# akosiorek/attend_infer_repeat

Measured on AMD Instinct MI355X. Metric: images/sec (train step, ELBO backward) multi-MNIST 50x50, 3-step AIR, higher is better.
Workload: dtype f32; 1 GPU; multi-MNIST-shaped 50x50 canvas, max_steps=3, glimpse 20x20, batch=64 per GPU, fp32, hipGraph replay (BASELINE configs[1]); global_batch=64, batch_per_gpu=64, parallelism=dp1, hipgraph=True, steps_per_graph_replay=1, keep_canvas_steps=True, collective=none, dist_world_size=1, params_finite_after_run=True, replicas_in_sync_after_run=True

## Files before the change

### attend_infer_repeat_amd/csrc/air_common.h

```cpp
#pragma once
#include <hip/hip_runtime.h>
#include <stdint.h>
#include <stdlib.h>
#include <mutex>
#include "../../include/air_hip.h"

#define AIR_WAVE 64

#define AIR_REQUIRE(cond, code) do { if (!(cond)) return (code); } while (0)
#define AIR_LAUNCH_CHECK() do { hipError_t e__ = hipGetLastError(); if (e__ != hipSuccess) return (int)e__; } while (0)

static inline long air_gemm_wide_min_tiles() {
    static const long wide_min = getenv("AIR_GEMM_WIDE_MIN_TILES") ? atol(getenv("AIR_GEMM_WIDE_MIN_TILES")) : 1000;
    return wide_min;
}
static inline int air_gemm_latency_tile(long tiles16) { return tiles16 > 1536 ? 32 : 16; }
static inline bool air_gemm_long_k(int M, int N, int K) { return K >= 512 && K >= 8 * (M < N ? M : N); }
static inline bool air_gemm_lone_on_tile16_kw4(int M, int N, int K) {
    const long t = (long)((M + 15) / 16) * ((N + 15) / 16);
    return t <= air_gemm_wide_min_tiles() && air_gemm_latency_tile(t) == 16 && !air_gemm_long_k(M, N, K);
}

static inline hipStream_t air_stream(void *s) { return reinterpret_cast<hipStream_t>(s); }
static inline bool air_aligned16(const void *p) { return (reinterpret_cast<uintptr_t>(p) & 15u) == 0; }
__device__ __forceinline__ bool air_aligned16_dev(const void *p) { return (reinterpret_cast<uintptr_t>(p) & 15u) == 0; }
static inline int air_cdiv(long a, long b) { return (int)((a + b - 1) / b); }
static inline size_t air_rider_blocks(size_t nq, int nth, size_t cap) {
    static const double qpt = getenv("AIR_RIDER_QPT") ? atof(getenv("AIR_RIDER_QPT")) : 2.0;
    const double per_wg = (qpt > 0.05 ? qpt : 2.0) * nth;
    size_t extra = (size_t)(((double)nq + per_wg - 1.0) / per_wg);
    return extra > cap ? cap : extra;
}
template <typename K>
static inline int air_resident_grid(K kernel, int threads, size_t lds, int fallback) {
    struct Entry { const void *k; int threads; size_t lds; int dev; int grid; };
    static Entry cache[32];
    static int n_cached = 0;
    static std::mutex mu;
    int dev = 0;
    if (hipGetDevice(&dev) != hipSuccess) return fallback;
    const void *key = reinterpret_cast<const void *>(kernel);
    std::lock_guard<std::mutex> lock(mu);
    for (int i = 0; i < n_cached; ++i)
        if (cache[i].k == key && cache[i].threads == threads && cache[i].lds == lds && cache[i].dev == dev) return cache[i].grid;
    int per_cu = 0, cus = 0;
    if (hipDeviceGetAttribute(&cus, hipDeviceAttributeMultiprocessorCount, dev) != hipSuccess ||
        hipOccupancyMaxActiveBlocksPerMultiprocessor(&per_cu, kernel, threads, lds) != hipSuccess || per_cu < 1 || cus < 1)
        return fallback;
    if (n_cached < 32) cache[n_cached++] = Entry{key, threads, lds, dev, per_cu * cus};
    return per_cu * cus;
}

__device__ __forceinline__ int opaque_zero() {
    int z;
    asm volatile("v_mov_b32 %0, 0" : "=v"(z));
    return z;
}

__device__ __forceinline__ float wave_sum(float v) {
#pragma unroll
    for (int off = 32; off > 0; off >>= 1) v += __shfl_down(v, off, 64);
    return v;
}
__device__ __forceinline__ double wave_sum(double v) {
#pragma unroll
    for (int off = 32; off > 0; off >>= 1) v += __shfl_down(v, off, 64);
    return v;
}
__device__ __forceinline__ float wave_sum_all(float v) {
#pragma unroll
    for (int off = 32; off > 0; off >>= 1) v += __shfl_xor(v, off, 64);
    return v;
}
__device__ __forceinline__ double wave_sum_all(double v) {
#pragma unroll
    for (int off = 32; off > 0; off >>= 1) v += __shfl_xor(v, off, 64);
    return v;
}
__device__ __forceinline__ float wave_max_all(float v) {
#pragma unroll
    for (int off = 32; off > 0; off >>= 1) v = fmaxf(v, __shfl_xor(v, off, 64));
    return v;
}

template <typename T>
__device__ __forceinline__ T wave_reduce8(const T (&v)[8]) {
    const int lane = threadIdx.x & 63;
    const bool h5 = (lane & 32) != 0, h4 = (lane & 16) != 0, h3 = (lane & 8) != 0;
    T a[4], b[2];
#pragma unroll
    for (int i = 0; i < 4; ++i) a[i] = (h5 ? v[i + 4] : v[i]) + __shfl_xor(h5 ? v[i] : v[i + 4], 32, 64);
#pragma unroll
    for (int i = 0; i < 2; ++i) b[i] = (h4 ? a[i + 2] : a[i]) + __shfl_xor(h4 ? a[i] : a[i + 2], 16, 64);
    T c = (h3 ? b[1] : b[0]) + __shfl_xor(h3 ? b[0] : b[1], 8, 64);
    c += __shfl_xor(c, 4, 64);
    c += __shfl_xor(c, 2, 64);
    c += __shfl_xor(c, 1, 64);
    return c;
}
__device__ __forceinline__ int wave_reduce8_slot() {
    const int lane = threadIdx.x & 63;
    return ((lane >> 5) & 1) * 4 + ((lane >> 4) & 1) * 2 + ((lane >> 3) & 1);
}

template <int NV>
__device__ __forceinline__ void block_sum(float (&v)[NV], float *scratch) {
    const int lane = threadIdx.x & 63, wid = threadIdx.x >> 6, nw = (blockDim.x + 63) >> 6;
#pragma unroll
    for (int k = 0; k < NV; ++k) v[k] = wave_sum(v[k]);
    if (lane == 0) {
#pragma unroll
        for (int k = 0; k < NV; ++k) scratch[wid * NV + k] = v[k];
    }
    __syncthreads();
    if (wid == 0) {
#pragma unroll
        for (int k = 0; k < NV; ++k) {
            float x = lane < nw ? scratch[lane * NV + k] : 0.f;
            v[k] = wave_sum(x);
        }
    }
}

__device__ __forceinline__ float lin_m11(int k, int n, double step) {
#pragma clang fp contract(off)
    if (n <= 1) return -1.0f;
    if (k == n - 1) return 1.0f;
    const double prod = (double)k * step;
    return (float)(prod + -1.0);
}
__device__ __forceinline__ float grid_coord(float s, float X, float t, float half_extent) {
#pragma clang fp contract(off)
    const float a = s * X;
    const float b = a + t;
    const float c = b + 1.0f;
    return c * half_extent;
}
__device__ __forceinline__ float4 attention_box4(const float4 w4, float Wf, float Hf) {
#pragma clang fp contract(off)
    float4 bx;
    bx.x = Wf * ((1.f - w4.x) + w4.y) * 0.5f;
    bx.y = Hf * ((1.f - w4.z) + w4.w) * 0.5f;
    bx.z = Wf * w4.x;
    bx.w = Hf * w4.z;
    return bx;
}
__device__ __forceinline__ float sigmoidf_(float x) { return 1.0f / (1.0f + __expf(-x)); }
__device__ __forceinline__ float sigmoid_acc(float x) { return 1.0f / (1.0f + expf(-x)); }
__device__ __forceinline__ float softplus_acc(float x) { return x > 20.0f ? x : log1pf(expf(x)); }
__device__ __forceinline__ float elu_acc(float x) { return x > 0.0f ? x : expm1f(x); }
```

### attend_infer_repeat_amd/csrc/gemm_kernels.hip

```cpp
#include "air_common.h"
#include "prologue_device.h"
#include "optimizer_device.h"
#include "engine_device.h"
#include "nvil_device.h"
#include "gemm_device.h"
#include <cstring>
#include <type_traits>


struct AproArgs {
    const float *A2, *a_bias;
    float *a_out;
    int a_elu;
};
#define AIR_OPT_MAX_RANGES 4
struct OptFold {
    float *p; const float *g0; float *ms, *mg, *mom;
    size_t n_model;
    const float *lr_dev;
    float lr_mult_tail, decay, momentum, eps, gscale;
    unsigned fold_mask;
    int n_ranges, tiles;
    size_t lo[AIR_OPT_MAX_RANGES], hi[AIR_OPT_MAX_RANGES];
    int64_t *gstep; uint64_t *rng_state; uint64_t rng_inc;
};
#define AIR_OPT_RIDERS(OPT_)                                                                                                     \
    if ((int)blockIdx.x >= OPT_.tiles) {                                                                                         \
        const int vb = (int)blockIdx.x - OPT_.tiles, vg = (int)gridDim.x - OPT_.tiles;                                           \
        for (int r = 0; r < OPT_.n_ranges; ++r) {                                                                                \
            RmspropSlice sl;                                                                                                     \
            sl.p = OPT_.p; sl.g = OPT_.g0; sl.ms = OPT_.ms; sl.mg = OPT_.mg; sl.mom = OPT_.mom;                                  \
            sl.lo = OPT_.lo[r]; sl.hi = OPT_.hi[r]; sl.n_model = OPT_.n_model; sl.lr_dev = OPT_.lr_dev;                          \
            sl.lr_mult_tail = OPT_.lr_mult_tail; sl.decay = OPT_.decay; sl.momentum = OPT_.momentum; sl.eps = OPT_.eps;          \
            sl.gscale = OPT_.gscale;                                                                                             \
            rmsprop_slice_body(sl, vb, vg);                                                                                      \
        }                                                                                                                        \
        if (vb == 0 && threadIdx.x == 0) {                                                                                       \
            if (OPT_.gstep) OPT_.gstep[0] += 1;                                                                                  \
            if (OPT_.rng_state) OPT_.rng_state[1] += OPT_.rng_inc;                                                               \
        }                                                                                                                        \
        return;                                                                                                                  \
    }
struct GaussEpi {
    const float *pre, *eps, *loc, *scale, *dkl_row;
    float *dpre;
    int ld_pre, ld_dpre, D;
    float raw_offset, pl, ps, dkl_scale, guard;
    unsigned mask;
};
struct GatherArgs {
    const float *data, *obs;
    float *obs_out;
    long long n_items;
    int item_floats, shuffle, B;
    const uint64_t *seed;
    const int64_t *step;
    int64_t *idx_out;
    unsigned copy_mask;
};
__device__ __forceinline__ long long gather_item(const GatherArgs &gt, int m) {
    const unsigned long long ctr = (unsigned long long)gt.step[0] * (unsigned long long)gt.B + (unsigned long long)m;
    if (gt.shuffle) {
        uint32_t r[4];
        philox4x32(ctr, 1, gt.seed[0], r);
        const unsigned long long wide = ((unsigned long long)r[0] << 32) | r[1];
        return (long long)(((unsigned __int128)wide * (unsigned __int128)gt.n_items) >> 64);
    }
    return (long long)(ctr % (unsigned long long)gt.n_items);
}
struct GemmArgs {
    const float *A, *B, *bias, *aux;
    float *C, *colsum, *ws;
    int M, N, K, lda, ldb, ldc, ldaux;
    int ta, tb, epi, S, chunks_per_split, vecA, vecB;
    float beta;
};


__device__ __forceinline__ float apply_epilogue(float v, int m, int n, const GemmArgs &g) {
    if (g.beta != 0.f) v += g.beta * g.C[(size_t)m * g.ldc + n];
    switch (g.epi) {
        case AIR_EPI_BIAS: v += g.bias[n]; break;
        case AIR_EPI_BIAS_ELU: v = elu_acc(v + g.bias[n]); break;
        case AIR_EPI_MUL_DELU: {
            const float y = g.aux[(size_t)m * g.ldaux + n];
            v *= (y > 0.f ? 1.f : y + 1.f);
        } break;
        case AIR_EPI_ADD_AUX:
            v += g.aux[(size_t)m * g.ldaux + n];
            if (g.bias) v += g.bias[n];
            break;
        case AIR_EPI_ADD_AUX_ELU:
            v += g.aux[(size_t)m * g.ldaux + n];
            if (g.bias) v += g.bias[n];
            v = elu_acc(v);
            break;
        default: break;
    }
    return v;
}

template <int MT, int NT, int KW, bool BF, bool APRO = false, bool OPT = false, bool GBW = false, bool GATH = false>
__device__ __forceinline__ void gemm_body(const GemmArgs &g, const int block_tile, const int split, const AproArgs pro = AproArgs(),
                                          void *c16 = nullptr, const OptFold *opt = nullptr, const bool fold = false,
                                          const GaussEpi *gb = nullptr, const GatherArgs *gt = nullptr, const bool gcopy = false) {
    const gh_t hC = (gh_t)c16;
    constexpr int TM = 16 * MT, TN = 16 * NT;
    constexpr int NWN = (KW == 1) ? 4 : 1;
    constexpr int NWV = (KW == 1) ? 4 : KW;
    constexpr int NTH = 64 * NWV;
    constexpr int LDT = TN + 4;
    __shared__ float s_tile[NWV][TM * LDT];
    __shared__ float s_col[NWV][TN];

    const gcf gA = (gcf)g.A, gB = (gcf)g.B, gBias = (gcf)g.bias, gAux = (gcf)g.aux;
    const gf gC = (gf)g.C, gWs = (gf)g.ws, gCol = (gf)g.colsum;
    const int lane = threadIdx.x & 63, wave = threadIdx.x >> 6;
    const int li = lane & 15, lg = lane >> 4;
    const int tiles_n = (g.N + TN * NWN - 1) / (TN * NWN);
    const int tm = block_tile / tiles_n, tn = block_tile - tm * tiles_n;
    const int m0 = tm * TM;
    const int n0 = (tn * NWN + (KW == 1 ? wave : 0)) * TN;

    const int total_chunks = (g.K + 15) >> 4;
    const int c_begin = split * g.chunks_per_split;
    int c_end = c_begin + g.chunks_per_split;
    if (c_end > total_chunks) c_end = total_chunks;

    f32x4 acc[MT][NT];
#pragma unroll
    for (int a = 0; a < MT; ++a)
#pragma unroll
        for (int b = 0; b < NT; ++b) acc[a][b] = (f32x4){0.f, 0.f, 0.f, 0.f};
    float csum[NT];
#pragma unroll
    for (int b = 0; b < NT; ++b) csum[b] = 0.f;
    const bool want_colsum = (g.colsum != nullptr) && (tm == 0);

    int rowA[MT], colB[NT];
    bool okA[MT], okB[NT];
#pragma unroll
    for (int a = 0; a < MT; ++a) { rowA[a] = m0 + 16 * a + li; okA[a] = rowA[a] < g.M; }
#pragma unroll
    for (int b = 0; b < NT; ++b) { colB[b] = n0 + 16 * b + li; okB[b] = colB[b] < g.N; }

    constexpr int EPT = (KW > 1) ? (TM * TN + NTH - 1) / NTH : 1;
    float e_bias[EPT], e_aux[EPT], e_c[EPT];
    if (KW > 1 && g.S == 1) {
#pragma unroll
        for (int i = 0; i < EPT; ++i) {
            const int e = threadIdx.x + NTH * i;
            const int r = e / TN, cidx = e - r * TN;
            const int m = m0 + r, n = n0 + cidx;
            const bool ok = (e < TM * TN) && m < g.M && n < g.N;
            e_bias[i] = (ok && g.bias != nullptr) ? gBias[n] : 0.f;
            e_aux[i] = (ok && g.epi >= AIR_EPI_MUL_DELU) ? gAux[(size_t)m * g.ldaux + n] : 0.f;
            e_c[i] = (ok && g.beta != 0.f) ? gC[(size_t)m * g.ldc + n] : 0.f;
        }
    }
    float b_loc[GBW ? EPT : 1], b_scale[GBW ? EPT : 1], b_eps[GBW ? EPT : 1], b_raw[GBW ? EPT : 1], b_dk[GBW ? EPT : 1];
    if (GBW && KW > 1 && fold) {
#pragma unroll
        for (int i = 0; i < EPT; ++i) {
            const int e = threadIdx.x + NTH * i;
            const int r = e / TN, cidx = e - r * TN;
            const int m = m0 + r, n = n0 + cidx;
            const bool ok = (e < TM * TN) && m < g.M && n < g.N;
            const size_t o = ok ? (size_t)m * gb->D + n : 0;
            b_loc[i] = ok ? ((gcf)gb->loc)[o] : 0.f;
            b_scale[i] = ok ? ((gcf)gb->scale)[o] : 1.f;
            b_eps[i] = ok ? ((gcf)gb->eps)[o] : 0.f;
            b_raw[i] = ok ? ((gcf)gb->pre)[(size_t)m * gb->ld_pre + gb->D + n] : 0.f;
            b_dk[i] = (ok && gb->dkl_row) ? ((gcf)gb->dkl_row)[m] : 0.f;
        }
    }
    float o_p[OPT ? EPT : 1], o_ms[OPT ? EPT : 1], o_mg[OPT ? EPT : 1], o_mom[OPT ? EPT : 1];
    float o_lr0 = 0.f;
    if (OPT && KW > 1 && fold) {
        o_lr0 = ((gcf)opt->lr_dev)[0];
#pragma unroll
        for (int i = 0; i < EPT; ++i) {
            const int e = threadIdx.x + NTH * i;
            const int r = e / TN, cidx = e - r * TN;
            const int m = m0 + r, n = n0 + cidx;
            const bool ok = (e < TM * TN) && m < g.M && n < g.N;
            const size_t idx = ok ? (size_t)((gC + (size_t)m * g.ldc + n) - (gf)opt->g0) : 0;
            o_p[i] = ok ? ((gf)opt->p)[idx] : 0.f;
            o_ms[i] = ok ? ((gf)opt->ms)[idx] : 0.f;
            o_mg[i] = ok ? ((gf)opt->mg)[idx] : 0.f;
            o_mom[i] = ok ? ((gf)opt->mom)[idx] : 0.f;
        }
    }

    const int c_step = (KW > 1) ? KW : 1;
    int c = c_begin + ((KW > 1) ? wave : 0);
    constexpr int U = (MT * NT == 1) ? (KW == 16 ? 10 : 8) : 4;
    int full_end = g.K >> 4;
    if (full_end > c_end) full_end = c_end;
    int rowAc[MT], colBc[NT];
#pragma unroll
    for (int a = 0; a < MT; ++a) rowAc[a] = okA[a] ? rowA[a] : g.M - 1;
#pragma unroll
    for (int b = 0; b < NT; ++b) colBc[b] = okB[b] ? colB[b] : g.N - 1;
    const int gcol = GATH ? (int)(gA - (gcf)gt->obs) : 0;
    const gcf gAs = GATH ? (gcf)gt->data + gcol : gA;
    const int ldAs = GATH ? gt->item_floats : g.lda;
    int rowAs[MT];
#pragma unroll
    for (int a = 0; a < MT; ++a) rowAs[a] = GATH ? (int)gather_item(*gt, rowAc[a]) : rowAc[a];
    if (GATH && gcopy && tn == 0 && split == 0 && wave == 0 && lg == 0 && gt->idx_out && gcol == 0) {
#pragma unroll
        for (int a = 0; a < MT; ++a) if (okA[a]) gt->idx_out[rowA[a]] = rowAs[a];
    }
#pragma nounroll
    for (; c < full_end; c += U * c_step) {
        f32x4 fa[U][MT], fb[U][NT];
        f32x4 fa2[APRO ? U : 1][APRO ? MT : 1], fab[APRO ? U : 1];
#pragma unroll
        for (int u = 0; u < U; ++u) {
            const int cu = c + u * c_step;
            if (cu < full_end) {
                const int k = (cu << 4) + 4 * lg;
#pragma unroll
                for (int a = 0; a < MT; ++a) {
                    fa[u][a] = g.ta ? ld_kstrided_full(gA, g.lda, rowAc[a], k)
                                    : ld_kcontig_full(gAs, ldAs, rowAs[a], k, g.vecA != 0);
                    if (APRO) {
                        fa2[u][a] = ld_kcontig_full((gcf)pro.A2, g.lda, rowAc[a], k, g.vecA != 0);
                        fab[u] = ld_kcontig_full((gcf)pro.a_bias, 0, 0, k, g.vecA != 0);
                    }
                }
#pragma unroll
                for (int b = 0; b < NT; ++b)
                    fb[u][b] = g.tb ? ld_kcontig_full(gB, g.ldb, colBc[b], k, g.vecB != 0)
                                    : ld_kstrided_full(gB, g.ldb, colBc[b], k);
            } else {
#pragma unroll
                for (int a = 0; a < MT; ++a) fa[u][a] = (f32x4){0.f, 0.f, 0.f, 0.f};
#pragma unroll
                for (int b = 0; b < NT; ++b) fb[u][b] = (f32x4){0.f, 0.f, 0.f, 0.f};
            }
        }
#pragma unroll
        for (int u = 0; u < U; ++u) {
            if (c + u * c_step >= full_end) break;
            if (APRO) {
#pragma unroll
                for (int a = 0; a < MT; ++a) {
                    f32x4 v = (fa[u][a] + fa2[u][a]) + fab[u];
                    if (pro.a_elu) { v.x = elu_acc(v.x); v.y = elu_acc(v.y); v.z = elu_acc(v.z); v.w = elu_acc(v.w); }
                    fa[u][a] = v;
                    if (pro.a_out != nullptr && tn == 0 && okA[a])
                        *(f32x4 *)(pro.a_out + (size_t)rowA[a] * g.lda + (((c + u * c_step) << 4) + 4 * lg)) = v;
                }
            }
            if (GATH && gcopy && tn == 0) {
#pragma unroll
                for (int a = 0; a < MT; ++a)
                    if (okA[a]) *(f32x4 *)(gt->obs_out + (size_t)rowA[a] * g.lda + gcol + (((c + u * c_step) << 4) + 4 * lg)) = fa[u][a];
            }
            mfma_chunk<MT, NT, BF>(acc, fa[u], fb[u]);
            if (want_colsum) {
#pragma unroll
                for (int b = 0; b < NT; ++b)
                    csum[b] += okB[b] ? (fb[u][b].x + fb[u][b].y) + (fb[u][b].z + fb[u][b].w) : 0.f;
            }
        }
    }
    const int pc = g.K >> 4;
    if ((g.K & 15) && pc >= c_begin && pc < c_end && (KW == 1 || ((pc - c_begin) % KW) == wave)) {
        const int k = (pc << 4) + 4 * lg;
        f32x4 fa[MT], fb[NT];
#pragma unroll
        for (int a = 0; a < MT; ++a)
            fa[a] = g.ta ? ld_kstrided(gA, g.lda, rowA[a], okA[a], k, g.K)
                         : ld_kcontig(gAs, ldAs, GATH ? rowAs[a] : rowA[a], okA[a], k, g.K, g.vecA != 0);
        if (GATH && gcopy && tn == 0) {
#pragma unroll
            for (int a = 0; a < MT; ++a) {
                if (!okA[a]) continue;
                float *d = gt->obs_out + (size_t)rowA[a] * g.lda + gcol + k;
                if (k < g.K) d[0] = fa[a].x;
                if (k + 1 < g.K) d[1] = fa[a].y;
                if (k + 2 < g.K) d[2] = fa[a].z;
                if (k + 3 < g.K) d[3] = fa[a].w;
            }
        }
#pragma unroll
        for (int b = 0; b < NT; ++b)
            fb[b] = g.tb ? ld_kcontig(gB, g.ldb, colB[b], okB[b], k, g.K, g.vecB != 0)
                         : ld_kstrided(gB, g.ldb, colB[b], okB[b], k, g.K);
        mfma_chunk<MT, NT, BF>(acc, fa, fb);
        if (want_colsum) {
#pragma unroll
            for (int b = 0; b < NT; ++b) csum[b] += (fb[b].x + fb[b].y) + (fb[b].z + fb[b].w);
        }
    }

#pragma unroll
    for (int a = 0; a < MT; ++a)
#pragma unroll
        for (int b = 0; b < NT; ++b)
#pragma unroll
            for (int r = 0; r < 4; ++r) s_tile[wave][(16 * a + 4 * lg + r) * LDT + 16 * b + li] = acc[a][b][r];
    if (want_colsum) {
#pragma unroll
        for (int b = 0; b < NT; ++b) {
            float v = csum[b];
            v += __shfl_xor(v, 16, 64);
            v += __shfl_xor(v, 32, 64);
            if (lg == 0) s_col[wave][16 * b + li] = v;
        }
    }
    __syncthreads();

    if (KW > 1) {
#pragma unroll
        for (int i = 0; i < EPT; ++i) {
            const int e = threadIdx.x + NTH * i;
            if (e >= TM * TN) continue;
            const int r = e / TN, cidx = e - r * TN;
            const int m = m0 + r, n = n0 + cidx;
            if (m >= g.M || n >= g.N) continue;
            const int off = r * LDT + cidx;
            float v = 0.f;
#pragma unroll
            for (int q = 0; q < NWV; q += 4)
                v += (s_tile[q][off] + s_tile[q + 1][off]) + (s_tile[q + 2][off] + s_tile[q + 3][off]);
            if (g.S > 1) {
                gWs[((size_t)split * g.M + m) * g.N + n] = v;
            } else {
                if (g.beta != 0.f) v += g.beta * e_c[i];
                switch (g.epi) {
                    case AIR_EPI_BIAS: v += e_bias[i]; break;
                    case AIR_EPI_BIAS_ELU: v = elu_acc(v + e_bias[i]); break;
                    case AIR_EPI_MUL_DELU: v *= (e_aux[i] > 0.f ? 1.f : e_aux[i] + 1.f); break;
                    case AIR_EPI_ADD_AUX: v += e_aux[i] + e_bias[i]; break;
                    case AIR_EPI_ADD_AUX_ELU: v = elu_acc(v + e_aux[i] + e_bias[i]); break;
                    default: break;
                }
                gC[(size_t)m * g.ldc + n] = v;
                if (BF && hC) hC[(size_t)m * g.ldc + n] = bf16_bits(v);
                if (GBW && fold) {
                    float dloc, draw;
                    gauss_bwd_elem(v, true, b_eps[i], b_loc[i], b_scale[i], gb->pl, gb->ps, b_dk[i] * gb->dkl_scale,
                                   b_raw[i] + gb->raw_offset, 0, n, gb->guard, dloc, draw);
                    const gf dp_ = (gf)gb->dpre + (size_t)m * gb->ld_dpre;
                    dp_[n] = dloc; dp_[gb->D + n] = draw;
                }
                if (OPT && fold) {
                    const size_t idx = (size_t)((gC + (size_t)m * g.ldc + n) - (gf)opt->g0);
                    const float lr = idx < opt->n_model ? o_lr0 : o_lr0 * opt->lr_mult_tail;
                    float pv = o_p[i], a = o_ms[i], b = o_mg[i], c = o_mom[i];
                    rmsprop_elem(pv, v, a, b, c, lr, opt->decay, opt->momentum, opt->eps, opt->gscale);
                    ((gf)opt->ms)[idx] = a; ((gf)opt->mg)[idx] = b; ((gf)opt->mom)[idx] = c; ((gf)opt->p)[idx] = pv;
                }
            }
        }
        if (want_colsum && threadIdx.x < TN) {
            const int n = n0 + threadIdx.x;
            if (n < g.N) {
                float v = 0.f;
#pragma unroll
                for (int q = 0; q < NWV; q += 4)
                    v += (s_col[q][threadIdx.x] + s_col[q + 1][threadIdx.x]) + (s_col[q + 2][threadIdx.x] + s_col[q + 3][threadIdx.x]);
                gCol[n] = v;
                if (OPT && fold) {
                    const size_t idx = (size_t)((gCol + n) - (gf)opt->g0);
                    const float lr = idx < opt->n_model ? o_lr0 : o_lr0 * opt->lr_mult_tail;
                    float pv = ((gf)opt->p)[idx], a = ((gf)opt->ms)[idx], b = ((gf)opt->mg)[idx], c = ((gf)opt->mom)[idx];
                    rmsprop_elem(pv, v, a, b, c, lr, opt->decay, opt->momentum, opt->eps, opt->gscale);
                    ((gf)opt->ms)[idx] = a; ((gf)opt->mg)[idx] = b; ((gf)opt->mom)[idx] = c; ((gf)opt->p)[idx] = pv;
                }
            }
        }
    } else {
        for (int e = lane; e < TM * TN; e += 64) {
            const int r = e / TN, cidx = e - r * TN;
            const int m = m0 + r, n = n0 + cidx;
            if (m >= g.M || n >= g.N) continue;
            const float v = s_tile[wave][r * LDT + cidx];
            if (g.S > 1) gWs[((size_t)split * g.M + m) * g.N + n] = v;
            else {
                const float o = apply_epilogue(v, m, n, g);
                gC[(size_t)m * g.ldc + n] = o;
                if (BF && hC) hC[(size_t)m * g.ldc + n] = bf16_bits(o);
            }
        }
        if (want_colsum && lane < TN) {
            const int n = n0 + lane;
            if (n < g.N) gCol[n] = s_col[wave][lane];
        }
    }
}

template <int MT, int NT, int KW, bool BF>
__global__ __launch_bounds__(KW == 1 ? 256 : 64 * KW) void gemm_f32_mfma_kernel(GemmArgs g) {
    gemm_body<MT, NT, KW, BF>(g, blockIdx.x, blockIdx.y);
}
template <int MT, int NT, int KW>
__global__ __launch_bounds__(KW == 1 ? 256 : 64 * KW) void gemm_bf16_c16_kernel(GemmArgs g, void *c16) {
    gemm_body<MT, NT, KW, true>(g, blockIdx.x, blockIdx.y, AproArgs(), c16);
}
template <int MT, int NT, int KW, bool BF>
__global__ __launch_bounds__(KW == 1 ? 256 : 64 * KW) void gemm_f32_mfma_apro_kernel(GemmArgs g, AproArgs pro) {
    gemm_body<MT, NT, KW, BF, true>(g, blockIdx.x, blockIdx.y, pro);
}

template <int MT, int KW, bool BF, bool TA, bool TB>
__device__ __forceinline__ void gemm_wide_body(const GemmArgs &g, const int block_tile) {
    constexpr int NT = 4, TM = 16 * MT, TN = 64;
    constexpr int NTH = 64 * KW;
    constexpr int LDT = TN + 4;
    static_assert(!TA || MT == 4, "an m-contiguous A operand is read 4 rows per lane: four interleaved row tiles");
    __shared__ float s_tile[KW][TM * LDT];
    __shared__ float s_col[KW][TN];

    const gcf gA = (gcf)g.A, gB = (gcf)g.B, gBias = (gcf)g.bias, gAux = (gcf)g.aux;
    const gf gC = (gf)g.C, gCol = (gf)g.colsum;
    const int lane = threadIdx.x & 63, wave = threadIdx.x >> 6;
    const int li = lane & 15, lg = lane >> 4;
    const int tiles_n = (g.N + TN - 1) / TN;
    const int tm = block_tile / tiles_n, tn = block_tile - tm * tiles_n;
    const int m0 = tm * TM, n0 = tn * TN;

    f32x4 acc[MT][NT];
#pragma unroll
    for (int a = 0; a < MT; ++a)
#pragma unroll
        for (int b = 0; b < NT; ++b) acc[a][b] = (f32x4){0.f, 0.f, 0.f, 0.f};
    float csum[NT] = {0.f, 0.f, 0.f, 0.f};
    const bool want_colsum = TA && (g.colsum != nullptr) && (tm == 0);

    int offA[TA ? 1 : MT], offB[TB ? NT : 1];
    if (TA) { int r = m0 + 4 * li; if (r > g.M - 4) r = g.M - 4; offA[0] = r; }
    else {
#pragma unroll
        for (int a = 0; a < MT; ++a) { int r = m0 + 16 * a + li; if (r > g.M - 1) r = g.M - 1; offA[a] = r * g.lda; }
    }
    if (!TB) { int c = n0 + 4 * li; if (c > g.N - 4) c = g.N - 4; offB[0] = c; }
    else {
#pragma unroll
        for (int b = 0; b < NT; ++b) { int c = n0 + 16 * b + li; if (c > g.N - 1) c = g.N - 1; offB[b] = c * g.ldb; }
    }

    constexpr int EPT = (TM * TN) / NTH;
    static_assert((TM * TN) % NTH == 0, "tile / threads");
    float e_bias[EPT], e_aux[EPT], e_c[EPT];
#pragma unroll
    for (int i = 0; i < EPT; ++i) {
        const int e = threadIdx.x + NTH * i;
        const int r = e / TN, cidx = e - r * TN;
        int m = m0 + r, n = n0 + cidx;
        if (m > g.M - 1) m = g.M - 1;
        if (n > g.N - 1) n = g.N - 1;
        e_bias[i] = g.bias != nullptr ? gBias[n] : 0.f;
        e_aux[i] = g.epi >= AIR_EPI_MUL_DELU ? gAux[(size_t)m * g.ldaux + n] : 0.f;
        e_c[i] = g.beta != 0.f ? gC[(size_t)m * g.ldc + n] : 0.f;
    }

    constexpr int U = (MT == 4) ? 3 : 4;
    const int full_end = g.K >> 4;
    auto load_chunk = [&](int k, f32x4 (&fa)[MT], f32x4 (&fb)[NT]) {
        if (TA) {
            f32x4 v[4];
#pragma unroll
            for (int j = 0; j < 4; ++j) v[j] = *(gcf4)(gA + (size_t)(k + j) * g.lda + offA[0]);
#pragma unroll
            for (int a = 0; a < MT; ++a) fa[a] = (f32x4){v[0][a], v[1][a], v[2][a], v[3][a]};
        } else {
#pragma unroll
            for (int a = 0; a < MT; ++a) fa[a] = *(gcf4)(gA + offA[a] + k);
        }
        if (!TB) {
// ... 248 lines not shown
                }
            }
        } else {
#pragma unroll
            for (int b = 0; b < NT; ++b) {
                if (full) {
                    if (B16) fb[b] = *(gcu4)(hB + offB[b] + k);
                    else fb[b] = pk8(*(gcf4)(gB + offB[b] + k), *(gcf4)(gB + offB[b] + k + 4));
                } else {
                    float v[8];
#pragma unroll
                    for (int j = 0; j < 8; ++j)
                        v[j] = j < kn ? (B16 ? bf16_to_f32(hB[offB[b] + k + j]) : gB[offB[b] + k + j]) : 0.f;
                    fb[b] = (u32x4){pk_bf16(v[0], v[1]), pk_bf16(v[2], v[3]), pk_bf16(v[4], v[5]), pk_bf16(v[6], v[7])};
                }
            }
        }
    };
    auto mma = [&](const u32x4 (&fa)[MT], const u32x4 (&fb)[NT]) {
#pragma unroll
        for (int a = 0; a < MT; ++a)
#pragma unroll
            for (int b = 0; b < NT; ++b)
                acc[a][b] = __builtin_amdgcn_mfma_f32_16x16x32_bf16(__builtin_bit_cast(bf16x8, fa[a]), __builtin_bit_cast(bf16x8, fb[b]),
                                                                   acc[a][b], 0, 0, 0);
    };

    constexpr int U = (MT == 4) ? ((A16 && B16) ? 2 : 1) : 2;
    const int full_end = g.K >> 5;
    int c = wave;
#pragma nounroll
    for (; c < full_end; c += U * KW) {
        u32x4 fa[U][MT], fb[U][NT];
#pragma unroll
        for (int u = 0; u < U; ++u) {
            int cu = c + u * KW;
            if (cu > full_end - 1) cu = full_end - 1;
            load_chunk((cu << 5) + 8 * lg, 8, fa[u], fb[u], true, c + u * KW < full_end);
        }
#pragma unroll
        for (int u = 0; u < U; ++u) {
            if (c + u * KW >= full_end) break;
            mma(fa[u], fb[u]);
        }
    }
    if ((g.K & 31) && (full_end % KW) == wave) {
        const int k = (full_end << 5) + 8 * lg;
        int kn = g.K - k;
        kn = kn < 0 ? 0 : (kn > 8 ? 8 : kn);
        u32x4 fa[MT], fb[NT];
        load_chunk(kn > 0 ? k : 0, kn, fa, fb, false, true);
        mma(fa, fb);
    }

#pragma unroll
    for (int a = 0; a < MT; ++a)
#pragma unroll
        for (int r = 0; r < 4; ++r) {
            const int row = TA ? 4 * (4 * lg + r) + a : 16 * a + 4 * lg + r;
            if (!TB) {
                *(f32x4 *)&s_tile[wave][row * LDT + 4 * li] = (f32x4){acc[a][0][r], acc[a][1][r], acc[a][2][r], acc[a][3][r]};
            } else {
#pragma unroll
                for (int b = 0; b < NT; ++b) s_tile[wave][row * LDT + 16 * b + li] = acc[a][b][r];
            }
        }
    if (want_colsum) {
#pragma unroll
        for (int b = 0; b < NT; ++b) {
            float v = csum[b];
            v += __shfl_xor(v, 16, 64);
            v += __shfl_xor(v, 32, 64);
            if (lg == 0) s_col[wave][TB ? 16 * b + li : 4 * li + b] = v;
        }
    }
    __syncthreads();
#pragma unroll
    for (int i = 0; i < EPT; ++i) {
        const int e = threadIdx.x + NTH * i;
        const int r = e / TN, cidx = e - r * TN;
        const int m = m0 + r, n = n0 + cidx;
        const int off = r * LDT + cidx;
        float v = 0.f;
#pragma unroll
        for (int q = 0; q < KW; q += 4) v += (s_tile[q][off] + s_tile[q + 1][off]) + (s_tile[q + 2][off] + s_tile[q + 3][off]);
        if (g.beta != 0.f) v += g.beta * e_c[i];
        switch (g.epi) {
            case AIR_EPI_BIAS: v += e_bias[i]; break;
            case AIR_EPI_BIAS_ELU: v = elu_acc(v + e_bias[i]); break;
            case AIR_EPI_MUL_DELU: v *= (e_aux[i] > 0.f ? 1.f : e_aux[i] + 1.f); break;
            case AIR_EPI_ADD_AUX: v += e_aux[i] + e_bias[i]; break;
            case AIR_EPI_ADD_AUX_ELU: v = elu_acc(v + e_aux[i] + e_bias[i]); break;
            default: break;
        }
        if (m < g.M && n < g.N) {
            gC[(size_t)m * g.ldc + n] = v;
            if (hC) hC[(size_t)m * g.ldc + n] = bf16_bits(v);
        }
    }
    if (want_colsum && threadIdx.x < TN) {
        const int n = n0 + threadIdx.x;
        if (n < g.N) {
            float v = 0.f;
#pragma unroll
            for (int q = 0; q < KW; q += 4)
                v += (s_col[q][threadIdx.x] + s_col[q + 1][threadIdx.x]) + (s_col[q + 2][threadIdx.x] + s_col[q + 3][threadIdx.x]);
            gCol[n] = v;
        }
    }
}
template <int MT, int KW, bool TA, bool TB, bool A16, bool B16>
__global__ __launch_bounds__(64 * KW) void gemm_wide16_kernel(GemmArgs g, Gemm16Ptrs h) {
    __shared__ Wide16Lds<MT, KW> lds;
    gemm_wide16_body<MT, KW, TA, TB, A16, B16>(g, h, blockIdx.x, lds);
}

#define AIR_GEMM_GROUP_MAX 8
struct GroupArgs {
    GemmArgs g[AIR_GEMM_GROUP_MAX];
    int tile_start[AIR_GEMM_GROUP_MAX + 1];
    int count;
    int xcd_map;
    unsigned sk_mask;
};
#define AIR_GROUP_LOCATE(P_, GA_, VB_)                                                                                           \
    int P_ = 0;                                                                                                                  \
    _Pragma("unroll")                                                                                                            \
    for (int i = 1; i < AIR_GEMM_GROUP_MAX; ++i)                                                                                 \
        if (i < GA_.count && VB_ >= GA_.tile_start[i]) P_ = i;                                                                   \
    P_ = __builtin_amdgcn_readfirstlane(P_)
#define AIR_GROUP_SWITCH(P_, CASE_)                                                                                              \
    switch (P_) {                                                                                                                \
        case 0: CASE_(0); break;                                                                                                 \
        case 1: CASE_(1); break;                                                                                                 \
        case 2: CASE_(2); break;                                                                                                 \
        case 3: CASE_(3); break;                                                                                                 \
        case 4: CASE_(4); break;                                                                                                 \
        case 5: CASE_(5); break;                                                                                                 \
        case 6: CASE_(6); break;                                                                                                 \
        default: CASE_(7); break;                                                                                                \
    }
#define AIR_GROUP_DISPATCH(GA_, VB_, CASE_)                                                                                      \
    do {                                                                                                                         \
        AIR_GROUP_LOCATE(p, GA_, VB_);                                                                                           \
        AIR_GROUP_SWITCH(p, CASE_);                                                                                              \
    } while (0)
template <int MT, int NT, int KW, bool BF>
__global__ __launch_bounds__(KW == 1 ? 256 : 64 * KW) void gemm_grouped_kernel(GroupArgs ga) {
#define AIR_GG_CASE(I_) gemm_body<MT, NT, KW, BF>(ga.g[I_], (int)blockIdx.x - ga.tile_start[I_], blockIdx.y)
    AIR_GROUP_DISPATCH(ga, (int)blockIdx.x, AIR_GG_CASE);
#undef AIR_GG_CASE
}

__global__ __launch_bounds__(1024) void gemm_grouped_gather_kernel(GroupArgs ga, GatherArgs gt) {
#define AIR_GG_CASE(I_)                                                                                                             \
    gemm_body<1, 1, 16, false, false, false, false, true>(ga.g[I_], (int)blockIdx.x - ga.tile_start[I_], blockIdx.y, AproArgs(), nullptr, \
                                                          nullptr, false, nullptr, &gt, cp)
    AIR_GROUP_LOCATE(p, ga, (int)blockIdx.x);
    const bool cp = (gt.copy_mask >> p) & 1u;
    AIR_GROUP_SWITCH(p, AIR_GG_CASE);
#undef AIR_GG_CASE
}

template <int MT, int NT, int KW, bool BF>
__global__ __launch_bounds__(KW == 1 ? 256 : 64 * KW) void gemm_grouped_opt_kernel(GroupArgs ga, OptFold opt) {
    AIR_OPT_RIDERS(opt);
#define AIR_OPT_CASE(I_)                                                                                                          \
    gemm_body<MT, NT, KW, BF, false, true>(ga.g[I_], (int)blockIdx.x - ga.tile_start[I_], blockIdx.y, AproArgs(), nullptr, &opt,  \
                                           ((opt.fold_mask >> I_) & 1u) != 0)
    AIR_GROUP_DISPATCH(ga, (int)blockIdx.x, AIR_OPT_CASE);
#undef AIR_OPT_CASE
}

template <bool OPT>
__device__ __forceinline__ void shortk_dw_body(const GemmArgs &g, const int vb, const int vg, const OptFold *opt, const bool fold) {
    const gcf gA = (gcf)g.A, gB = (gcf)g.B;
    const gf gC = (gf)g.C, gCol = (gf)g.colsum;
    const int lane = threadIdx.x & 63, wave = threadIdx.x >> 6, li = lane & 15, lg = lane >> 4;
    const int n_base = 64 * wave;
    if (n_base >= g.N) return;
    const int nch = g.K >> 4;
    f32x4 fb[4][4];
#pragma unroll
    for (int c = 0; c < 4; ++c)
#pragma unroll
        for (int t = 0; t < 4; ++t)
            fb[c][t] = c < nch ? ld_kstrided_full(gB, g.ldb, n_base + 16 * t + li, (c << 4) + 4 * lg) : (f32x4){0.f, 0.f, 0.f, 0.f};
    float o_lr0 = 0.f;
    if (OPT && fold) o_lr0 = ((gcf)opt->lr_dev)[0];
    if (gCol != nullptr && vb == 0) {
#pragma unroll
        for (int t = 0; t < 4; ++t) {
            float v = 0.f;
#pragma unroll
            for (int c = 0; c < 4; ++c) v += (fb[c][t].x + fb[c][t].y) + (fb[c][t].z + fb[c][t].w);
            v += __shfl_xor(v, 16, 64);
            v += __shfl_xor(v, 32, 64);
            if (lg == 0) {
                const int n = n_base + 16 * t + li;
                gCol[n] = v;
                if (OPT && fold) {
                    const size_t idx = (size_t)((gCol + n) - (gf)opt->g0);
                    const float lr = idx < opt->n_model ? o_lr0 : o_lr0 * opt->lr_mult_tail;
                    float pv = ((gf)opt->p)[idx], a = ((gf)opt->ms)[idx], b = ((gf)opt->mg)[idx], cmo = ((gf)opt->mom)[idx];
                    rmsprop_elem(pv, v, a, b, cmo, lr, opt->decay, opt->momentum, opt->eps, opt->gscale);
                    ((gf)opt->ms)[idx] = a; ((gf)opt->mg)[idx] = b; ((gf)opt->mom)[idx] = cmo; ((gf)opt->p)[idx] = pv;
                }
            }
        }
    }
    const int tiles_m = (g.M + 15) >> 4;
    int mt = vb;
    if (mt >= tiles_m) return;
    f32x4 fa[4];
    {
        int m = (mt << 4) + li; if (m > g.M - 1) m = g.M - 1;
#pragma unroll
        for (int c = 0; c < 4; ++c) fa[c] = c < nch ? ld_kstrided_full(gA, g.lda, m, (c << 4) + 4 * lg) : (f32x4){0.f, 0.f, 0.f, 0.f};
    }
#pragma nounroll
    for (; mt < tiles_m; mt += vg) {
        f32x4 fn[4];
        {
            int mn = ((mt + vg) << 4) + li; if (mn > g.M - 1) mn = g.M - 1;
#pragma unroll
            for (int c = 0; c < 4; ++c) fn[c] = c < nch ? ld_kstrided_full(gA, g.lda, mn, (c << 4) + 4 * lg) : (f32x4){0.f, 0.f, 0.f, 0.f};
        }
        const int mrow0 = (mt << 4) + 4 * lg;
        f32x4 o_p[4], o_ms[4], o_mg[4], o_mom[4];
#pragma unroll
        for (int t = 0; t < 4; ++t) { o_p[t] = (f32x4){0.f, 0.f, 0.f, 0.f}; o_ms[t] = o_p[t]; o_mg[t] = o_p[t]; o_mom[t] = o_p[t]; }
        if (OPT && fold) {
#pragma unroll
            for (int r = 0; r < 4; ++r) {
                int mr = mrow0 + r; if (mr > g.M - 1) mr = g.M - 1;
                const size_t idx0 = (size_t)((gC + (size_t)mr * g.ldc + n_base + li) - (gf)opt->g0);
#pragma unroll
                for (int t = 0; t < 4; ++t) {
                    o_p[t][r] = ((gf)opt->p)[idx0 + 16 * t]; o_ms[t][r] = ((gf)opt->ms)[idx0 + 16 * t];
                    o_mg[t][r] = ((gf)opt->mg)[idx0 + 16 * t]; o_mom[t][r] = ((gf)opt->mom)[idx0 + 16 * t];
                }
            }
        }
        f32x4 acc[4];
#pragma unroll
        for (int t = 0; t < 4; ++t) acc[t] = (f32x4){0.f, 0.f, 0.f, 0.f};
#pragma unroll
        for (int c = 0; c < 4; ++c)
#pragma unroll
            for (int j = 0; j < 4; ++j)
#pragma unroll
                for (int t = 0; t < 4; ++t) acc[t] = __builtin_amdgcn_mfma_f32_16x16x4f32(fa[c][j], fb[c][t][j], acc[t], 0, 0, 0);
#pragma unroll
        for (int t = 0; t < 4; ++t)
#pragma unroll
            for (int r = 0; r < 4; ++r) {
                const int mr = mrow0 + r;
                if (mr < g.M) {
                    const size_t off = (size_t)mr * g.ldc + n_base + 16 * t + li;
                    const float v = acc[t][r];
                    gC[off] = v;
                    if (OPT && fold) {
                        const size_t idx = (size_t)((gC + off) - (gf)opt->g0);
                        const float lr = idx < opt->n_model ? o_lr0 : o_lr0 * opt->lr_mult_tail;
                        float pv = o_p[t][r], a = o_ms[t][r], b = o_mg[t][r], cmo = o_mom[t][r];
                        rmsprop_elem(pv, v, a, b, cmo, lr, opt->decay, opt->momentum, opt->eps, opt->gscale);
                        ((gf)opt->ms)[idx] = a; ((gf)opt->mg)[idx] = b; ((gf)opt->mom)[idx] = cmo; ((gf)opt->p)[idx] = pv;
                    }
                }
            }
#pragma unroll
        for (int c = 0; c < 4; ++c) fa[c] = fn[c];
    }
}
static inline bool shortk_eligible(const AirGemmDesc &d) {
    static const int on = getenv("AIR_GEMM_SHORTK") ? atoi(getenv("AIR_GEMM_SHORTK")) : 1;
    static const int min_m = getenv("AIR_GEMM_SHORTK_MIN_M") ? atoi(getenv("AIR_GEMM_SHORTK_MIN_M")) : 4096;
    return on && d.ta && !d.tb && d.precision == AIR_PREC_F32 && d.K >= 16 && d.K <= 64 && d.K % 16 == 0 && d.N >= 64 && d.N <= 256 &&
           d.N % 64 == 0 && d.M >= min_m && d.epilogue == AIR_EPI_NONE && d.beta == 0.f && !d.A2 && !d.C16 && !d.bias;
}
static inline int shortk_workgroups(int M) {
    static const int cap = getenv("AIR_GEMM_SHORTK_WGS") ? atoi(getenv("AIR_GEMM_SHORTK_WGS")) : 384;
    const int t = air_cdiv(M, 16);
    return t < cap ? t : (cap < 1 ? 1 : cap);
}

template <int MT, int NT>
__global__ __launch_bounds__(256) void gemm_grouped_sk_kernel(GroupArgs ga) {
#define AIR_SK_CASE(I_)                                                                                                        \
    do {                                                                                                                       \
        if ((ga.sk_mask >> I_) & 1u)                                                                                           \
            shortk_dw_body<false>(ga.g[I_], (int)blockIdx.x - ga.tile_start[I_], ga.tile_start[I_ + 1] - ga.tile_start[I_], nullptr, false); \
        else gemm_body<MT, NT, 4, false>(ga.g[I_], (int)blockIdx.x - ga.tile_start[I_], blockIdx.y);                           \
    } while (0)
    AIR_GROUP_DISPATCH(ga, (int)blockIdx.x, AIR_SK_CASE);
#undef AIR_SK_CASE
}
__global__ __launch_bounds__(256) void gemm_grouped_opt_sk_kernel(GroupArgs ga, OptFold opt) {
    AIR_OPT_RIDERS(opt);
#define AIR_SK_CASE(I_)                                                                                                        \
    shortk_dw_body<true>(ga.g[I_], (int)blockIdx.x - ga.tile_start[I_], ga.tile_start[I_ + 1] - ga.tile_start[I_], &opt,        \
                         ((opt.fold_mask >> I_) & 1u) != 0)
    AIR_GROUP_DISPATCH(ga, (int)blockIdx.x, AIR_SK_CASE);
#undef AIR_SK_CASE
}

// ... 203 lines not shown
    gemm_single_form(M, N, K, colsum != nullptr, ws != nullptr, ws_bytes, f);
    g.S = f.S; g.chunks_per_split = f.chunks_per_split;
    hipStream_t st = air_stream(stream);
    if (f.KW == 1) return launch_gemm<2, 2, 1, BF>(g, st);
    return launch_gemm<1, 1, 4, BF>(g, st);
}

extern "C" int air_gemm(int ta, int tb, int M, int N, int K, const float *A, int lda, const float *B, int ldb,
                        float *C, int ldc, const float *bias, int epilogue, const float *aux, int ldaux, float beta,
                        float *colsum, void *ws, size_t ws_bytes, void *stream) {
    return gemm_dispatch<false>(ta, tb, M, N, K, A, lda, B, ldb, C, ldc, bias, epilogue, aux, ldaux, beta, colsum, ws,
                                ws_bytes, stream);
}
extern "C" int air_gemm_bf16(int ta, int tb, int M, int N, int K, const float *A, int lda, const float *B, int ldb,
                             float *C, int ldc, const float *bias, int epilogue, const float *aux, int ldaux, float beta,
                             float *colsum, void *ws, size_t ws_bytes, void *stream) {
    return gemm_dispatch<true>(ta, tb, M, N, K, A, lda, B, ldb, C, ldc, bias, epilogue, aux, ldaux, beta, colsum, ws,
                               ws_bytes, stream);
}

static int fill_gemm_args(GemmArgs &g, const AirGemmDesc &d) {
    AIR_REQUIRE(d.A && d.B && d.C, AIR_E_NULL);
    AIR_REQUIRE(d.M > 0 && d.N > 0 && d.K > 0, AIR_E_SHAPE);
    AIR_REQUIRE(d.lda >= (d.ta ? d.M : d.K) && d.ldb >= (d.tb ? d.K : d.N) && d.ldc >= d.N, AIR_E_SHAPE);
    AIR_REQUIRE(d.epilogue >= AIR_EPI_NONE && d.epilogue <= AIR_EPI_ADD_AUX_ELU, AIR_E_UNSUPPORTED);
    if (d.epilogue == AIR_EPI_BIAS || d.epilogue == AIR_EPI_BIAS_ELU) AIR_REQUIRE(d.bias, AIR_E_NULL);
    if (d.epilogue >= AIR_EPI_MUL_DELU) AIR_REQUIRE(d.aux && d.ldaux >= d.N, AIR_E_NULL);
    AIR_REQUIRE(!d.colsum || d.ta, AIR_E_UNSUPPORTED);
    if (d.A2) {
        AIR_REQUIRE(!d.ta && d.a_bias && (d.K % 16 == 0) && (d.lda % 4 == 0), AIR_E_UNSUPPORTED);
        AIR_REQUIRE(air_aligned16(d.A) && air_aligned16(d.A2) && air_aligned16(d.a_bias) && (!d.a_out || air_aligned16(d.a_out)),
                    AIR_E_ALIGN);
    }
    g.A = d.A; g.B = d.B; g.C = d.C; g.bias = d.bias; g.aux = d.aux; g.colsum = d.colsum; g.ws = nullptr;
    g.M = d.M; g.N = d.N; g.K = d.K; g.lda = d.lda; g.ldb = d.ldb; g.ldc = d.ldc; g.ldaux = d.ldaux;
    g.ta = d.ta ? 1 : 0; g.tb = d.tb ? 1 : 0; g.epi = d.epilogue; g.beta = d.beta;
    g.vecA = (!d.ta && (d.lda % 4 == 0) && air_aligned16(d.A)) ? 1 : 0;
    g.vecB = (d.tb && (d.ldb % 4 == 0) && air_aligned16(d.B)) ? 1 : 0;
    g.S = 1; g.chunks_per_split = (d.K + 15) / 16;
    return AIR_OK;
}

template <class GA, class Tiles>
static int group_tile_starts(GA &ga, const AirGemmDesc *descs, int count, Tiles tiles_of) {
    constexpr int MAX = (int)(sizeof(ga.g) / sizeof(ga.g[0]));
    int tiles = 0;
    for (int i = 0; i < count; ++i) {
        ga.tile_start[i] = tiles;
        const int t = tiles_of(i, descs[i]);
        if (t < 0) return t;
        tiles += t;
    }
    for (int i = count; i <= MAX; ++i) ga.tile_start[i] = tiles;
    return tiles;
}
static int accept_any(int, const AirGemmDesc &) { return AIR_OK; }
template <class GA, class Accept, class Tiles>
static int fill_group(GA &ga, const AirGemmDesc *descs, int count, Accept accept, Tiles tiles_of, int *total) {
    constexpr int MAX = (int)(sizeof(ga.g) / sizeof(ga.g[0]));
    const int tiles = group_tile_starts(ga, descs, count, [&](int i, const AirGemmDesc &d) {
        int st = accept(i, d);
        if (st == AIR_OK) st = fill_gemm_args(ga.g[i], d);
        return st ? st : tiles_of(i, d);
    });
    if (tiles < 0) return tiles;
    for (int i = count; i < MAX; ++i) ga.g[i] = ga.g[0];
    ga.count = count;
    ga.xcd_map = 0;
    if constexpr (std::is_same<GA, GroupArgs>::value) ga.sk_mask = 0;
    *total = tiles;
    return AIR_OK;
}
template <class GA16, class GA, class Mirrors>
static void group_to16(GA16 &g16, const GA &ga, Mirrors mirrors_of) {
    constexpr int MAX = (int)(sizeof(ga.g) / sizeof(ga.g[0]));
    for (int i = 0; i < MAX; ++i) {
        const int j = i < ga.count ? i : 0;
        g16.g[i] = ga.g[j];
        g16.h[i] = mirrors_of(j);
    }
    for (int i = 0; i <= MAX; ++i) g16.tile_start[i] = ga.tile_start[i];
    g16.count = ga.count; g16.xcd_map = ga.xcd_map;
}
static bool bf16_storage() {
    static const int use16 = getenv("AIR_GEMM_BF16_STORAGE") ? atoi(getenv("AIR_GEMM_BF16_STORAGE")) : 1;
    return use16 != 0;
}
static inline bool mirror_usable(const void *m16, int ld) { return m16 && ld % 2 == 0 && ((uintptr_t)m16 % 4 == 0); }

static long group_tiles16(const AirGemmDesc *descs, int count, unsigned skip_mask) {
    long tiles16 = 0;
    for (int i = 0; i < count; ++i)
        if (!((skip_mask >> i) & 1u)) tiles16 += (long)air_cdiv(descs[i].M, 16) * air_cdiv(descs[i].N, 16);
    return tiles16;
}
static inline int latency_tile(long tiles16) { return air_gemm_latency_tile(tiles16); }
static bool group_long_k(const AirGemmDesc *descs, int count, long tiles16) {
    bool long_k = tiles16 <= 1024;
    for (int i = 0; i < count; ++i) long_k = long_k && air_gemm_long_k(descs[i].M, descs[i].N, descs[i].K);
    return long_k;
}
static int problem_precision(const AirGemmDesc &d, bool bf) {
    AIR_REQUIRE(d.precision == AIR_PREC_F32 || d.precision == AIR_PREC_BF16, AIR_E_UNSUPPORTED);
    AIR_REQUIRE((d.precision == AIR_PREC_BF16) == bf, AIR_E_UNSUPPORTED);
    return AIR_OK;
}
static int group_precision(const AirGemmDesc *descs, int count, bool *bf) {
    *bf = descs[0].precision == AIR_PREC_BF16;
    for (int i = 0; i < count; ++i)
        if (int st = problem_precision(descs[i], *bf)) return st;
    return AIR_OK;
}

static long wide_min_tiles() { return air_gemm_wide_min_tiles(); }
static bool group_on_long_k_body(const AirGemmDesc *descs, int count, long tiles16) {
    return tiles16 <= wide_min_tiles() && group_long_k(descs, count, tiles16);
}
static bool wide_group_eligible(const AirGemmDesc *descs, int count, long tiles16, bool bf, int *min_k_out, bool *nt_short_out) {
    static const long wide_tn_bf = getenv("AIR_GEMM_WIDE_TN_BF16") ? atol(getenv("AIR_GEMM_WIDE_TN_BF16")) : 48;
    static const long wide_tn_f32 = getenv("AIR_GEMM_WIDE_TN_F32") ? atol(getenv("AIR_GEMM_WIDE_TN_F32")) : 48;
    static const long wide_nt_k = getenv("AIR_GEMM_WIDE_NT_K") ? atol(getenv("AIR_GEMM_WIDE_NT_K")) : 512;
    bool ok = tiles16 > wide_min_tiles();
    const int ta = descs[0].ta ? 1 : 0, tb = descs[0].tb ? 1 : 0;
    long tiles64 = 0;
    int min_k = 1 << 30;
    for (int i = 0; i < count && ok; ++i) {
        const AirGemmDesc &d = descs[i];
        ok = ok && (d.ta ? 1 : 0) == ta && (d.tb ? 1 : 0) == tb && !(ta && tb) && !d.A2;
        ok = ok && air_aligned16(d.B) && d.ldb % 4 == 0 && (!ta || d.K % 4 == 0) && (!tb || d.K % 4 == 0);
        ok = ok && d.M >= 4 && d.N >= 4 && d.K >= 4 && (!ta || d.M % 4 == 0) && (tb || d.N % 4 == 0);
        if (tiles16 <= 2048) ok = ok && air_aligned16(d.A) && d.lda % 4 == 0 && d.K % 4 == 0;
        tiles64 += (long)air_cdiv(d.M, 64) * air_cdiv(d.N, 64);
        if (d.K < min_k) min_k = d.K;
    }
    if (ok && ta) ok = tiles64 >= (bf ? wide_tn_bf : wide_tn_f32) && min_k >= 256;
    const bool nt_short = !ta && tb && min_k < wide_nt_k;
    if (ok && nt_short) ok = bf && tiles16 > 2048;
    *min_k_out = min_k; *nt_short_out = nt_short;
    return ok;
}
static bool wide_regime_weight_gradients(const AirGemmDesc *descs, int count, long tiles16) {
    int min_k = 1 << 30;
    bool all_tn = true;
    for (int i = 0; i < count; ++i) { all_tn = all_tn && descs[i].ta && !descs[i].tb; if (descs[i].K < min_k) min_k = descs[i].K; }
    return tiles16 > wide_min_tiles() && all_tn && min_k >= 256;
}

static int validate_group(const AirGemmDesc *descs, int count) {
    GemmArgs scratch;
    for (int i = 0; i < count; ++i)
        if (int st = fill_gemm_args(scratch, descs[i])) return st;
    return AIR_OK;
}
static int form_workgroups_of(const AirGemmForm &f, int i, const AirGemmDesc &d) {
    switch (f.family) {
        case AIR_GEMM_FAM_BIG: case AIR_GEMM_FAM_BIG16:
            return ((f.small_mask >> i) & 1u) ? air_cdiv(d.M, 16) * air_cdiv(d.N, 16) : air_cdiv(d.M, 64) * air_cdiv(d.N, 64);
        case AIR_GEMM_FAM_WIDE: case AIR_GEMM_FAM_WIDE16:
            return air_cdiv(d.M, 16 * f.MT) * air_cdiv(d.N, 64);
        case AIR_GEMM_FAM_SHORTK:
            if ((f.sk_mask >> i) & 1u) return shortk_workgroups(d.M);
            [[fallthrough]];
        default:
            return air_cdiv(d.M, f.tile) * air_cdiv(d.N, f.tile);
    }
}
static void form_sum_workgroups(AirGemmForm &f, const AirGemmDesc *descs, int count) {
    f.workgroups = 0;
    for (int i = 0; i < count; ++i) f.workgroups += form_workgroups_of(f, i, descs[i]);
}
static int big_tn_form(const AirGemmDesc *descs, int count, AirGemmForm &f) {
    AIR_REQUIRE(count <= AIR_GEMM_BIG_GROUP_MAX, AIR_E_SHAPE);
    const bool bf = descs[0].precision == AIR_PREC_BF16;
    int min_k = 1 << 30, n_wide = 0;
    GemmArgs scratch;
    for (int i = 0; i < count; ++i) {
        const AirGemmDesc &d = descs[i];
        if (int e = problem_precision(d, bf)) return e;
        AIR_REQUIRE(!d.A2, AIR_E_UNSUPPORTED);
        if (int e = fill_gemm_args(scratch, d)) return e;
        const bool wide = d.ta && !d.tb && air_aligned16(d.B) && d.ldb % 4 == 0 && d.K % 4 == 0 && d.M >= 4 && d.N >= 4 &&
                          d.M % 4 == 0 && d.N % 4 == 0;
        if (wide) {
            if (d.K < min_k) min_k = d.K;
            ++n_wide;
        } else f.small_mask |= 1u << i;
        if (bf && bf16_storage() && mirror_usable(d.A16, d.lda)) f.a16_mask |= 1u << i;
        if (bf && bf16_storage() && mirror_usable(d.B16, d.ldb)) f.b16_mask |= 1u << i;
    }
    AIR_REQUIRE(n_wide > 0, AIR_E_UNSUPPORTED);
    static const int big_xcd = getenv("AIR_GEMM_BIG_XCD") ? atoi(getenv("AIR_GEMM_BIG_XCD")) : 1;
    f.xcd_map = (big_xcd && min_k >= 1024) ? (bf ? 2 : 1) : 0;
    f.family = bf ? AIR_GEMM_FAM_BIG16 : AIR_GEMM_FAM_BIG;
    f.grouped = 1; f.MT = 4; f.KW = 8; f.bf = bf ? 1 : 0; f.ta = 1; f.tb = 0;
    f.threads = 512;
    form_sum_workgroups(f, descs, count);
    return AIR_OK;
}
static int launch_big_tn_group(const AirGemmDesc *descs, int count, const AirGemmForm &f, void *stream) {
    BigGroupArgs ga;
    int wt = 0;
    int st = fill_group(ga, descs, count, accept_any, [&](int i, const AirGemmDesc &d) { return form_workgroups_of(f, i, d); }, &wt);
    if (st) return st;
    ga.small_mask = f.small_mask;
    ga.xcd_map = f.xcd_map;
    hipStream_t stm = air_stream(stream);
    if (f.family == AIR_GEMM_FAM_BIG16) {
        BigGroupArgs16 g16;
        group_to16(g16, ga, [&](int j) {
            const AirGemmDesc &d = descs[j];
            return Gemm16Ptrs{((f.a16_mask >> j) & 1u) ? d.A16 : nullptr, ((f.b16_mask >> j) & 1u) ? d.B16 : nullptr, nullptr};
        });
        g16.small_mask = ga.small_mask;
        hipLaunchKernelGGL((gemm_big_group_wide16_tn_kernel<4, 8>), dim3(wt), dim3(512), 0, stm, g16);
    } else hipLaunchKernelGGL((gemm_big_group_wide_tn_kernel<4, 8, false>), dim3(wt), dim3(512), 0, stm, ga);
    AIR_LAUNCH_CHECK();
    return AIR_OK;
}

static unsigned shortk_mask(const AirGemmDesc *descs, int count) {
    unsigned m = 0;
    for (int i = 0; i < count; ++i) {
        if (descs[i].A2 || descs[i].C16 || descs[i].precision != AIR_PREC_F32) return 0;
        if (shortk_eligible(descs[i])) m |= 1u << i;
    }
    return m;
}
static int launch_grouped_sk(const AirGemmDesc *descs, int count, const AirGemmForm &f, void *stream) {
    GroupArgs ga;
    int tiles = 0;
    int err = fill_group(ga, descs, count, accept_any, [&](int i, const AirGemmDesc &d) { return form_workgroups_of(f, i, d); }, &tiles);
    if (err) return err;
    ga.sk_mask = f.sk_mask;
    hipStream_t st = air_stream(stream);
    if (f.MT == 1) hipLaunchKernelGGL((gemm_grouped_sk_kernel<1, 1>), dim3(tiles), dim3(256), 0, st, ga);
    else hipLaunchKernelGGL((gemm_grouped_sk_kernel<2, 2>), dim3(tiles), dim3(256), 0, st, ga);
    AIR_LAUNCH_CHECK();
    return AIR_OK;
}

extern "C" int air_gemm_grouped_gather_fits(const AirGemmDesc *descs, int count, const AirBatchGather *g) {
    if (!descs || !g || count < 1 || count > AIR_GEMM_GROUP_MAX) return 0;
    if (!g->dataset || !g->obs || !g->seed_dev || !g->step_dev || g->n_items <= 0 || g->item_floats <= 0 || g->B <= 0) return 0;
    if (g->item_floats % 4 || !air_aligned16(g->dataset) || !air_aligned16(g->obs)) return 0;
    long tiles16 = 0;
    for (int i = 0; i < count; ++i) {
        const AirGemmDesc &d = descs[i];
        if (d.ta || d.A2 || d.C16 || d.precision != AIR_PREC_F32 || d.M != g->B || d.lda != g->item_floats) return 0;
        const long off = (const float *)d.A - (const float *)g->obs;
        if (off < 0 || off + d.K > g->item_floats || off % 4) return 0;
        tiles16 += (long)air_cdiv(d.M, 16) * air_cdiv(d.N, 16);
    }
    return group_on_long_k_body(descs, count, tiles16) ? 1 : 0;
}
extern "C" int air_gemm_grouped_gather(const AirGemmDesc *descs, int count, const AirBatchGather *g, void *stream) {
    AIR_REQUIRE(descs && g, AIR_E_NULL);
    AIR_REQUIRE(air_gemm_grouped_gather_fits(descs, count, g) == 1, AIR_E_UNSUPPORTED);
    GroupArgs ga;
    int tiles = 0;
    int err = fill_group(ga, descs, count, accept_any, [&](int i, const AirGemmDesc &d) {
        ga.g[i].vecA = 1;
        return air_cdiv(d.M, 16) * air_cdiv(d.N, 16);
    }, &tiles);
    if (err) return err;
    const GatherArgs gt = {g->dataset, g->obs, g->obs, g->n_items, g->item_floats, g->shuffle ? 1 : 0, g->B, g->seed_dev, g->step_dev,
                           g->idx_out, g->copy_mask};
    hipLaunchKernelGGL(gemm_grouped_gather_kernel, dim3(tiles), dim3(1024), 0, air_stream(stream), ga, gt);
    AIR_LAUNCH_CHECK();
    return AIR_OK;
}

static int gemm_grouped_form(const AirGemmDesc *descs, int count, AirGemmForm &f) {
    memset(&f, 0, sizeof f);
    if (count > AIR_GEMM_GROUP_MAX) return big_tn_form(descs, count, f);
    AIR_REQUIRE(count > 0 && count <= AIR_GEMM_GROUP_MAX, AIR_E_SHAPE);
    f.grouped = count > 1 ? 1 : 0;
    if (const unsigned skm = shortk_mask(descs, count)) {
        if (int err = validate_group(descs, count)) return err;
        f.family = AIR_GEMM_FAM_SHORTK; f.grouped = 1; f.sk_mask = skm;
        f.tile = latency_tile(group_tiles16(descs, count, skm));
        f.MT = f.NT = f.tile == 16 ? 1 : 2; f.KW = 4; f.threads = 256;
        form_sum_workgroups(f, descs, count);
        return AIR_OK;
    }
    const long tiles16 = group_tiles16(descs, count, 0u);
    const int T_ = latency_tile(tiles16);
    if (int err = validate_group(descs, count)) return err;
    const bool long_k = group_long_k(descs, count, tiles16);
    bool bf;
    if (int err = group_precision(descs, count, &bf)) return err;
    f.bf = bf ? 1 : 0;
    {
        const int ta = descs[0].ta ? 1 : 0, tb = descs[0].tb ? 1 : 0;
        int min_k;
        bool nt_short;
        const bool ok = wide_group_eligible(descs, count, tiles16, bf, &min_k, &nt_short);
        if (ok && bf && ta) {
            memset(&f, 0, sizeof f);
            return big_tn_form(descs, count, f);
        }
        if (ok) {
            f.family = bf ? AIR_GEMM_FAM_WIDE16 : AIR_GEMM_FAM_WIDE;
            f.ta = ta; f.tb = tb; f.nt_short = nt_short ? 1 : 0;
            f.MT = ta ? 4 : (nt_short ? 2 : 1); f.KW = 8; f.threads = 512;
            form_sum_workgroups(f, descs, count);
            f.xcd_map = (ta && min_k >= 1024) ? 1 : 0;
            if (bf) {
                bool a16 = bf16_storage(), b16 = bf16_storage();
                for (int i = 0; i < count; ++i) {
                    a16 = a16 && mirror_usable(descs[i].A16, descs[i].lda);
                    b16 = b16 && mirror_usable(descs[i].B16, descs[i].ldb);
                }
                f.a16_mask = a16 ? (1u << count) - 1u : 0u;
                f.b16_mask = b16 ? (1u << count) - 1u : 0u;
            }
            return AIR_OK;
        }
    }
    for (int i = 0; i < count; ++i) AIR_REQUIRE(!descs[i].A2 || count == 1, AIR_E_UNSUPPORTED);
    bool any_c16 = false;
    for (int i = 0; i < count; ++i) any_c16 = any_c16 || (descs[i].C16 != nullptr);
    f.tile = T_; f.long_k = long_k ? 1 : 0;
    f.MT = f.NT = (long_k || T_ == 16) ? 1 : 2; f.KW = long_k ? 16 : 4; f.threads = 64 * f.KW;
    if (any_c16) {
        AIR_REQUIRE(bf && !descs[0].A2, AIR_E_UNSUPPORTED);
        f.family = AIR_GEMM_FAM_C16;
    } else if (count == 1 && descs[0].A2) {
        AIR_REQUIRE(T_ == 16, AIR_E_UNSUPPORTED);
        f.family = AIR_GEMM_FAM_APRO; f.MT = f.NT = 1; f.KW = 4; f.threads = 256;
    } else f.family = AIR_GEMM_FAM_TILE;
    form_sum_workgroups(f, descs, count);
    return AIR_OK;
}
extern "C" int air_gemm_grouped_form(const AirGemmDesc *descs, int count, AirGemmForm *out) {
    AIR_REQUIRE(descs && out, AIR_E_NULL);
    return gemm_grouped_form(descs, count, *out);
}

extern "C" int air_gemm_grouped(const AirGemmDesc *descs, int count, void *stream) {
    AIR_REQUIRE(descs, AIR_E_NULL);
    AirGemmForm f;
    if (int err = gemm_grouped_form(descs, count, f)) return err;
    if (f.family == AIR_GEMM_FAM_BIG || f.family == AIR_GEMM_FAM_BIG16) return launch_big_tn_group(descs, count, f, stream);
    if (f.family == AIR_GEMM_FAM_SHORTK) return launch_grouped_sk(descs, count, f, stream);
    GroupArgs ga;
    int tiles = 0;
    const bool wide = f.family == AIR_GEMM_FAM_WIDE || f.family == AIR_GEMM_FAM_WIDE16;
    int err = fill_group(ga, descs, count, accept_any, [&](int i, const AirGemmDesc &d) { return form_workgroups_of(f, i, d); }, &tiles);
    if (err) return err;
    hipStream_t st = air_stream(stream);
    const bool bf = f.bf != 0;
    if (wide) {
        const int wt = tiles;
        ga.xcd_map = f.xcd_map;
        if (bf) {
            const bool a16 = f.a16_mask != 0u, b16 = f.b16_mask != 0u;
            GroupArgs16 g16;
            group_to16(g16, ga, [&](int j) {
                return Gemm16Ptrs{a16 ? descs[j].A16 : nullptr, b16 ? descs[j].B16 : nullptr, descs[j].C16};
            });
#define AIR_WIDE16_LAUNCH2(MT_, TA_, TB_, A16_, B16_)                                                                              \
            do {                                                                                                           \
                if (!f.grouped) hipLaunchKernelGGL((gemm_wide16_kernel<MT_, 8, TA_, TB_, A16_, B16_>), dim3(wt), dim3(512), 0, st, g16.g[0], g16.h[0]); \
                else hipLaunchKernelGGL((gemm_grouped_wide16_kernel<MT_, 8, TA_, TB_, A16_, B16_>), dim3(wt), dim3(512), 0, st, g16);                   \
            } while (0)
#define AIR_WIDE16_LAUNCH(MT_, TA_, TB_)                                                                                   \
            do {                                                                                                           \
                if (a16 && b16) AIR_WIDE16_LAUNCH2(MT_, TA_, TB_, true, true);                                             \
                else if (a16) AIR_WIDE16_LAUNCH2(MT_, TA_, TB_, true, false);                                              \
                else if (b16) AIR_WIDE16_LAUNCH2(MT_, TA_, TB_, false, true);                                              \
                else AIR_WIDE16_LAUNCH2(MT_, TA_, TB_, false, false);                                                      \
            } while (0)
            if (f.MT == 4) AIR_WIDE16_LAUNCH(4, true, false);
            else if (f.MT == 2) AIR_WIDE16_LAUNCH(2, false, true);
            else if (f.tb) AIR_WIDE16_LAUNCH(1, false, true);
            else AIR_WIDE16_LAUNCH(1, false, false);
#undef AIR_WIDE16_LAUNCH
#undef AIR_WIDE16_LAUNCH2
            AIR_LAUNCH_CHECK();
            return AIR_OK;
        }
#define AIR_WIDE_LAUNCH(MT_, TA_, TB_)                                                                                     \
        do {                                                                                                               \
            if (!f.grouped) hipLaunchKernelGGL((gemm_wide_kernel<MT_, 8, false, TA_, TB_>), dim3(wt), dim3(512), 0, st, ga.g[0]);         \
            else hipLaunchKernelGGL((gemm_grouped_wide_kernel<MT_, 8, false, TA_, TB_>), dim3(wt), dim3(512), 0, st, ga);                 \
        } while (0)
        if (f.MT == 4) AIR_WIDE_LAUNCH(4, true, false);
        else if (f.MT == 2) AIR_WIDE_LAUNCH(2, false, true);
        else if (f.tb) AIR_WIDE_LAUNCH(1, false, true);
        else AIR_WIDE_LAUNCH(1, false, false);
#undef AIR_WIDE_LAUNCH
        AIR_LAUNCH_CHECK();
        return AIR_OK;
    }
#define AIR_TILE_FORMS(LAUNCH_)                                                                                      \
    do {                                                                                                             \
        if (f.KW == 16) LAUNCH_(1, 1, 16, 1024);                                                                     \
        else if (f.MT == 1) LAUNCH_(1, 1, 4, 256);                                                                   \
        else LAUNCH_(2, 2, 4, 256);                                                                                  \
    } while (0)
#define AIR_GROUP_LAUNCH(MT_, NT_, KW_, NTH_)                                                                        \
    do {                                                                                                             \
        if (bf) hipLaunchKernelGGL((gemm_grouped_kernel<MT_, NT_, KW_, true>), dim3(tiles), dim3(NTH_), 0, st, ga);   \
        else hipLaunchKernelGGL((gemm_grouped_kernel<MT_, NT_, KW_, false>), dim3(tiles), dim3(NTH_), 0, st, ga);     \
    } while (0)
#define AIR_SINGLE_LAUNCH(MT_, NT_, KW_, NTH_)                                                                       \
    do {                                                                                                             \
        if (bf) hipLaunchKernelGGL((gemm_f32_mfma_kernel<MT_, NT_, KW_, true>), dim3(tiles, 1), dim3(NTH_), 0, st, ga.g[0]);  \
        else hipLaunchKernelGGL((gemm_f32_mfma_kernel<MT_, NT_, KW_, false>), dim3(tiles, 1), dim3(NTH_), 0, st, ga.g[0]);    \
    } while (0)
    if (f.family == AIR_GEMM_FAM_C16) {
        C16Ptrs c16;
        for (int i = 0; i < AIR_GEMM_GROUP_MAX; ++i) c16.p[i] = i < count ? descs[i].C16 : nullptr;
#define AIR_C16_LAUNCH(MT_, NT_, KW_, NTH_)                                                                          \
        do {                                                                                                         \
            if (!f.grouped) hipLaunchKernelGGL((gemm_bf16_c16_kernel<MT_, NT_, KW_>), dim3(tiles, 1), dim3(NTH_), 0, st, ga.g[0], c16.p[0]);  \
            else hipLaunchKernelGGL((gemm_grouped_c16_kernel<MT_, NT_, KW_>), dim3(tiles), dim3(NTH_), 0, st, ga, c16);                     \
        } while (0)
        AIR_TILE_FORMS(AIR_C16_LAUNCH);
#undef AIR_C16_LAUNCH
    } else if (f.family == AIR_GEMM_FAM_APRO) {
        const AproArgs pro = {descs[0].A2, descs[0].a_bias, descs[0].a_out, descs[0].a_elu};
        if (bf) hipLaunchKernelGGL((gemm_f32_mfma_apro_kernel<1, 1, 4, true>), dim3(tiles, 1), dim3(256), 0, st, ga.g[0], pro);
        else hipLaunchKernelGGL((gemm_f32_mfma_apro_kernel<1, 1, 4, false>), dim3(tiles, 1), dim3(256), 0, st, ga.g[0], pro);
    } else if (!f.grouped) AIR_TILE_FORMS(AIR_SINGLE_LAUNCH);
    else AIR_TILE_FORMS(AIR_GROUP_LAUNCH);
#undef AIR_SINGLE_LAUNCH
#undef AIR_GROUP_LAUNCH
#undef AIR_TILE_FORMS
    AIR_LAUNCH_CHECK();
    return AIR_OK;
}

extern "C" int air_gemm_grouped_gauss_bwd(const AirGemmDesc *descs, int count, const AirGaussBwdEpi *e, const float *imp_parts,
                                          int n_parts, float *imp_sum, const float *baseline, const float *logp, float *nvil_out,
                                          float *dlogp, float *dbaseline, int B, float *ema_dev, const float *kl_parts,
                                          int n_kl_parts, float *kl_row_out, int kl_rows, void *stream) {
    AIR_REQUIRE(descs && e, AIR_E_NULL);
    AIR_REQUIRE(count > 0 && count <= AIR_GEMM_GROUP_MAX && e->problem >= 0 && e->problem < count, AIR_E_SHAPE);
    AIR_REQUIRE(e->pre && e->eps && e->loc && e->scale && e->dpre && e->D > 0 && e->ld_pre >= 2 * e->D && e->ld_dpre >= 2 * e->D, AIR_E_NULL);
    AIR_REQUIRE(!imp_parts || (baseline && logp && nvil_out && B > 0 && n_parts > 0), AIR_E_NULL);
    AIR_REQUIRE(n_kl_parts >= 0 && (n_kl_parts == 0 || (kl_parts && kl_row_out && kl_rows > 0)), AIR_E_NULL);
    {
        const AirGemmDesc &d = descs[e->problem];
        AIR_REQUIRE(d.N == e->D && d.beta == 0.f && d.epilogue == AIR_EPI_NONE && !d.colsum, AIR_E_UNSUPPORTED);
    }
    GroupArgs ga;
    const long tiles16 = group_tiles16(descs, count, 0u);
    AIR_REQUIRE(tiles16 <= 1000, AIR_E_UNSUPPORTED);
    int tiles = 0;
    const bool bf = descs[0].precision == AIR_PREC_BF16;
    int err = fill_group(ga, descs, count,
        [&](int, const AirGemmDesc &d) -> int {
            if (int e = problem_precision(d, bf)) return e;
            AIR_REQUIRE(!d.A2 && !d.C16, AIR_E_UNSUPPORTED);
            return AIR_OK;
        },
        [&](int, const AirGemmDesc &d) { return air_cdiv(d.M, 16) * air_cdiv(d.N, 16); }, &tiles);
    if (err) return err;
    const bool long_k = group_long_k(descs, count, tiles16);
    GaussEpi gb;
    gb.pre = e->pre; gb.eps = e->eps; gb.loc = e->loc; gb.scale = e->scale; gb.dkl_row = e->dkl_row; gb.dpre = e->dpre;
    gb.ld_pre = e->ld_pre; gb.ld_dpre = e->ld_dpre; gb.D = e->D; gb.raw_offset = e->raw_offset; gb.pl = e->p_loc; gb.ps = e->p_scale;
    gb.dkl_scale = e->dkl_scale; gb.guard = e->guard_eps; gb.mask = 1u << e->problem;
    const NvilArgs nv = {imp_parts, baseline, logp, nvil_out, dlogp, dbaseline, B, n_parts > 0 ? n_parts : 1, imp_sum, ema_dev};
    const KlParts kp = {kl_parts, kl_row_out, n_kl_parts};
    const int riders = (imp_parts ? 1 : 0) + (n_kl_parts > 0 ? 1 : 0);
    hipStream_t st = air_stream(stream);
#define AIR_GB_LAUNCH(KW_, NTH_)                                                                                                   \
    do {                                                                                                                           \
        if (bf) hipLaunchKernelGGL((gemm_grouped_gb_kernel<1, 1, KW_, true>), dim3(tiles + riders), dim3(NTH_), 0, st, ga, gb, nv, kp, tiles, kl_rows);  \
        else hipLaunchKernelGGL((gemm_grouped_gb_kernel<1, 1, KW_, false>), dim3(tiles + riders), dim3(NTH_), 0, st, ga, gb, nv, kp, tiles, kl_rows);   \
    } while (0)
    if (long_k) AIR_GB_LAUNCH(16, 1024); else AIR_GB_LAUNCH(4, 256);
#undef AIR_GB_LAUNCH
    AIR_LAUNCH_CHECK();
    return AIR_OK;
}

extern "C" int air_gemm_grouped_opt(const AirGemmDesc *descs, int count, const AirOptFold *o, void *stream) {
    AIR_REQUIRE(descs && o, AIR_E_NULL);
    AIR_REQUIRE(count > 0 && count <= AIR_GEMM_GROUP_MAX, AIR_E_SHAPE);
    AIR_REQUIRE(o->p && o->g && o->ms && o->mg && o->mom && o->lr_dev, AIR_E_NULL);
    AIR_REQUIRE(o->n_ranges >= 0 && o->n_ranges <= AIR_OPT_MAX_RANGES && o->n_model % 4 == 0, AIR_E_SHAPE);
    AIR_REQUIRE(air_aligned16(o->p) && air_aligned16(o->g) && air_aligned16(o->ms) && air_aligned16(o->mg) && air_aligned16(o->mom), AIR_E_ALIGN);
    GroupArgs ga;
    const unsigned sk_mask = shortk_mask(descs, count);
    AIR_REQUIRE(sk_mask == 0 || sk_mask == (1u << count) - 1u, AIR_E_UNSUPPORTED);
    const long tiles16 = group_tiles16(descs, count, sk_mask);
    const int T_ = latency_tile(tiles16);
    int tiles = 0;
    const bool bf = descs[0].precision == AIR_PREC_BF16;
    int err = fill_group(ga, descs, count,
        [&](int, const AirGemmDesc &d) -> int {
            if (int e = problem_precision(d, bf)) return e;
            AIR_REQUIRE(!d.A2 && !d.C16, AIR_E_UNSUPPORTED);
            return AIR_OK;
        },
        [&](int i, const AirGemmDesc &d) -> int {
            if ((o->fold_mask >> i) & 1u) {
                AIR_REQUIRE(d.beta == 0.f && d.epilogue == AIR_EPI_NONE, AIR_E_UNSUPPORTED);
                AIR_REQUIRE(d.C >= o->g && (!d.colsum || d.colsum >= o->g), AIR_E_SHAPE);
            }
            return ((sk_mask >> i) & 1u) ? shortk_workgroups(d.M) : air_cdiv(d.M, T_) * air_cdiv(d.N, T_);
// ... 75 lines not shown
```

### attend_infer_repeat_amd/csrc/lstm_kernels.hip

```cpp
#include "air_common.h"
#include "prologue_device.h"
#include "optimizer_device.h"
#include "engine_device.h"
#include "nvil_device.h"
#include "gemm_device.h"

template <int KW, bool BF, bool B_KCONTIG>
__device__ __forceinline__ void tile16_kloop(f32x4 (&acc)[1][1], gcf gA, int lda, int rowA, bool okA, bool vecA, gcf gB,
                                             int ldb, int colB, bool okB, bool vecB, int K, int limA, int limB) {
    const int lane = threadIdx.x & 63, wave = threadIdx.x >> 6, lg = lane >> 4;
    constexpr int U = 4;
    const int full_end = K >> 4;
    const int rowAc = okA ? rowA : limA - 1, colBc = okB ? colB : limB;
#pragma nounroll
    for (int c = wave; c < full_end; c += U * KW) {
        f32x4 fa[U][1], fb[U][1];
#pragma unroll
        for (int u = 0; u < U; ++u) {
            const int cu = c + u * KW;
            if (cu < full_end) {
                const int k = (cu << 4) + 4 * lg;
                fa[u][0] = ld_kcontig_full(gA, lda, rowAc, k, vecA);
                fb[u][0] = B_KCONTIG ? ld_kcontig_full(gB, ldb, colBc, k, vecB) : ld_kstrided_full(gB, ldb, colBc, k);
            } else {
                fa[u][0] = (f32x4){0.f, 0.f, 0.f, 0.f};
                fb[u][0] = (f32x4){0.f, 0.f, 0.f, 0.f};
            }
        }
#pragma unroll
        for (int u = 0; u < U; ++u) {
            if (c + u * KW >= full_end) break;
            mfma_chunk<1, 1, BF>(acc, fa[u], fb[u]);
        }
    }
    const int pc = K >> 4;
    if ((K & 15) && (pc % KW) == wave) {
        const int k = (pc << 4) + 4 * lg;
        f32x4 fa[1], fb[1];
        fa[0] = ld_kcontig(gA, lda, rowA, okA, k, K, vecA);
        fb[0] = B_KCONTIG ? ld_kcontig(gB, ldb, colB, okB, k, K, vecB) : ld_kstrided(gB, ldb, colB, okB, k, K);
        mfma_chunk<1, 1, BF>(acc, fa, fb);
    }
}

template <int KW, bool BF>
__device__ __forceinline__ void tile16_kloop2(f32x4 (&acc0)[1][1], f32x4 (&acc1)[1][1], gcf gA0, int lda0, bool vecA0, gcf gB0, int K0,
                                              gcf gA1, int lda1, bool vecA1, gcf gB1, int K1, int ldb, int rowA, bool okA, int colB,
                                              bool okB, int limA, int limB) {
    const int lane = threadIdx.x & 63, wave = threadIdx.x >> 6, lg = lane >> 4;
    constexpr int U = 4;
    const int full0 = K0 >> 4, full1 = K1 >> 4;
    const int rowAc = okA ? rowA : limA - 1, colBc = okB ? colB : limB;
    const int fmax = full0 > full1 ? full0 : full1;
#pragma nounroll
    for (int c = wave; c < fmax; c += U * KW) {
        f32x4 fa0[U][1], fb0[U][1], fa1[U][1], fb1[U][1];
#pragma unroll
        for (int u = 0; u < U; ++u) {
            const int cu = c + u * KW;
            const int k = (cu << 4) + 4 * lg;
            if (cu < full0) { fa0[u][0] = ld_kcontig_full(gA0, lda0, rowAc, k, vecA0); fb0[u][0] = ld_kstrided_full(gB0, ldb, colBc, k); }
            else { fa0[u][0] = (f32x4){0.f, 0.f, 0.f, 0.f}; fb0[u][0] = (f32x4){0.f, 0.f, 0.f, 0.f}; }
            if (cu < full1) { fa1[u][0] = ld_kcontig_full(gA1, lda1, rowAc, k, vecA1); fb1[u][0] = ld_kstrided_full(gB1, ldb, colBc, k); }
            else { fa1[u][0] = (f32x4){0.f, 0.f, 0.f, 0.f}; fb1[u][0] = (f32x4){0.f, 0.f, 0.f, 0.f}; }
        }
#pragma unroll
        for (int u = 0; u < U; ++u) {
            if (c + u * KW < full0) mfma_chunk<1, 1, BF>(acc0, fa0[u], fb0[u]);
        }
#pragma unroll
        for (int u = 0; u < U; ++u) {
            if (c + u * KW < full1) mfma_chunk<1, 1, BF>(acc1, fa1[u], fb1[u]);
        }
    }
    const int pc0 = K0 >> 4, pc1 = K1 >> 4;
    if ((K0 & 15) && (pc0 % KW) == wave) {
        const int k = (pc0 << 4) + 4 * lg;
        f32x4 fa[1], fb[1];
        fa[0] = ld_kcontig(gA0, lda0, rowA, okA, k, K0, vecA0);
        fb[0] = ld_kstrided(gB0, ldb, colB, okB, k, K0);
        mfma_chunk<1, 1, BF>(acc0, fa, fb);
    }
    if ((K1 & 15) && (pc1 % KW) == wave) {
        const int k = (pc1 << 4) + 4 * lg;
        f32x4 fa[1], fb[1];
        fa[0] = ld_kcontig(gA1, lda1, rowA, okA, k, K1, vecA1);
        fb[0] = ld_kstrided(gB1, ldb, colB, okB, k, K1);
        mfma_chunk<1, 1, BF>(acc1, fa, fb);
    }
}

struct LstmFwdArgs {
    const float *h_prev, *w_h, *gx, *c_prev;
    float *h, *c, *gate_act;
    int M, Hd, ldw, ldgx, vecA;
    int ldh, ldc;
    int tiles;
    float fb;
};
template <bool BF>
__global__ __launch_bounds__(256) void lstm_fwd_fused_kernel(LstmFwdArgs g, PrologueArgs pro) {
    constexpr int KW = 4, LDT = 20;
    __shared__ float s_tile[KW][16 * LDT];
    if ((int)blockIdx.x >= g.tiles) {
        step_prologue_body(pro, (int)blockIdx.x - g.tiles, (int)gridDim.x - g.tiles);
        return;
    }
    const int lane = threadIdx.x & 63, wave = threadIdx.x >> 6, li = lane & 15, lg = lane >> 4;
    const int tiles_u = (g.Hd + 3) >> 2;
    const int tm = blockIdx.x / tiles_u, tu = blockIdx.x - tm * tiles_u;
    const int m0 = tm * 16, u0 = tu * 4;
    const int ub = u0 + (li & 3);
    const bool okB = ub < g.Hd;
    const int colB = (li >> 2) * g.Hd + ub;
    const int rowA = m0 + li;
    const bool okA = rowA < g.M;
    const int er = threadIdx.x >> 2, eu = u0 + (threadIdx.x & 3), em = m0 + er;
    const bool e_ok = threadIdx.x < 64 && em < g.M && eu < g.Hd;
    float e_gx[4] = {0.f, 0.f, 0.f, 0.f}, e_c = 0.f;
    if (e_ok) {
        const gcf gx = (gcf)g.gx + (size_t)em * g.ldgx + eu;
#pragma unroll
        for (int q = 0; q < 4; ++q) e_gx[q] = gx[(size_t)q * g.Hd];
        e_c = ((gcf)g.c_prev)[(size_t)em * g.ldc + eu];
    }
    f32x4 acc[1][1];
    acc[0][0] = (f32x4){0.f, 0.f, 0.f, 0.f};
    tile16_kloop<KW, BF, false>(acc, (gcf)g.h_prev, g.ldh, rowA, okA, g.vecA != 0, (gcf)g.w_h, g.ldw, colB, okB, false, g.Hd,
                                g.M, (li >> 2) * g.Hd + g.Hd - 1);
#pragma unroll
    for (int r = 0; r < 4; ++r) s_tile[wave][(4 * lg + r) * LDT + li] = acc[0][0][r];
    __syncthreads();
    if (e_ok) {
        float pre[4];
#pragma unroll
        for (int q = 0; q < 4; ++q) {
            const int off = er * LDT + 4 * q + (threadIdx.x & 3);
            pre[q] = ((s_tile[0][off] + s_tile[1][off]) + (s_tile[2][off] + s_tile[3][off])) + e_gx[q];
        }
        const float gi = sigmoid_acc(pre[0]);
        const float gj = tanhf(pre[1]);
        const float gf = sigmoid_acc(pre[2] + g.fb);
        const float go = sigmoid_acc(pre[3]);
        const float cn = gf * e_c + gi * gj;
        const size_t e = (size_t)em * g.Hd + eu;
        ((gf_t)g.c)[e] = cn;
        ((gf_t)g.h)[e] = tanhf(cn) * go;
        const gf_t ar = (gf_t)g.gate_act + (size_t)em * 4 * g.Hd + eu;
        ar[0] = gi; ar[g.Hd] = gj; ar[2 * (size_t)g.Hd] = gf; ar[3 * (size_t)g.Hd] = go;
    }
}

struct LstmFirstArgs { const float *x, *w_x, *b; float *gx_out; int E, ldx, vecX; };
template <bool BF>
__global__ __launch_bounds__(256) void lstm_fwd_first_kernel(LstmFwdArgs g, LstmFirstArgs f, PrologueArgs pro) {
    constexpr int KW = 4, LDT = 20;
    __shared__ float s_x[KW][16 * LDT], s_h[KW][16 * LDT];
    if ((int)blockIdx.x >= g.tiles) {
        step_prologue_body(pro, (int)blockIdx.x - g.tiles, (int)gridDim.x - g.tiles);
        return;
    }
    const int lane = threadIdx.x & 63, wave = threadIdx.x >> 6, li = lane & 15, lg = lane >> 4;
    const int tiles_u = (g.Hd + 3) >> 2;
    const int tm = blockIdx.x / tiles_u, tu = blockIdx.x - tm * tiles_u;
    const int m0 = tm * 16, u0 = tu * 4;
    const int ub = u0 + (li & 3);
    const bool okB = ub < g.Hd;
    const int colB = (li >> 2) * g.Hd + ub;
    const int rowA = m0 + li;
    const bool okA = rowA < g.M;
    const int er = threadIdx.x >> 2, eu = u0 + (threadIdx.x & 3), em = m0 + er;
    const bool e_ok = threadIdx.x < 64 && em < g.M && eu < g.Hd;
    float e_b[4] = {0.f, 0.f, 0.f, 0.f}, e_c = 0.f;
    if (e_ok) {
#pragma unroll
        for (int q = 0; q < 4; ++q) e_b[q] = ((gcf)f.b)[(size_t)q * g.Hd + eu];
// ... 79 lines not shown
            const int o0 = er * LDT + ed, o1 = o0 + 8;
            const float locp = ((s_tile[0][o0] + s_tile[1][o0]) + (s_tile[2][o0] + s_tile[3][o0])) + e_bl;
            const float raw = ((s_tile[0][o1] + s_tile[1][o1]) + (s_tile[2][o1] + s_tile[3][o1])) + e_br;
            const gf_t qr = (gf_t)g.q + (size_t)em * 2 * g.A;
            qr[ea] = locp; qr[g.A + ea] = raw;
            const float s = guard_scale(softplus_acc(raw + g.raw_offset), g.guard);
            const float v = locp + s * e_eps;
            const size_t o = (size_t)em * g.A + ea;
            ((gf_t)g.loc)[o] = locp; ((gf_t)g.scale)[o] = s; ((gf_t)g.what)[o] = v;
            const int t = em / g.B, bb = em - t * g.B;
            ((gf_t)g.pack)[(size_t)bb * width + t * g.A + ea] = v;
            kl = normal_kl(locp, s, g.pl, g.ps);
        }
        kl += __shfl_xor(kl, 1, 64);
        kl += __shfl_xor(kl, 2, 64);
        kl += __shfl_xor(kl, 4, 64);
        if (ed == 0 && em < g.M) ((gf_t)g.kl_parts)[(size_t)tn * g.M + em] = kl;
    }
}
extern "C" int air_what_head_parts(int A) { return (A + 7) / 8; }
extern "C" int air_what_head_fwd(const float *x, int ldx, int K, const float *w, const float *b, const float *eps, float raw_offset,
                                 float p_loc, float p_scale, float *q, float *loc, float *scale, float *sample, float *kl_parts,
                                 int A, const float *where, const float *presence, const float *state0, const float *state1,
                                 float *pack_out, int T, int B, int S0, int S1, float guard_eps, int precision, void *stream) {
    AIR_REQUIRE(x && w && b && eps && q && loc && scale && sample && kl_parts && where && presence && pack_out, AIR_E_NULL);
    AIR_REQUIRE((S0 == 0 || state0) && (S1 == 0 || state1), AIR_E_NULL);
    AIR_REQUIRE(T > 0 && B > 0 && A > 0 && K > 0 && ldx >= K && S0 >= 0 && S1 >= 0, AIR_E_SHAPE);
    AIR_REQUIRE(precision == AIR_PREC_F32 || precision == AIR_PREC_BF16, AIR_E_UNSUPPORTED);
    WhatHeadArgs g;
    g.x = x; g.w = w; g.b = b; g.eps = eps; g.q = q; g.loc = loc; g.scale = scale; g.what = sample; g.kl_parts = kl_parts; g.pack = pack_out;
    g.where = where; g.presence = presence; g.s0 = state0; g.s1 = state1;
    g.M = T * B; g.K = K; g.A = A; g.ldx = ldx; g.vecX = ((ldx % 4) == 0 && air_aligned16(x)) ? 1 : 0;
    g.T = T; g.B = B; g.S0 = S0; g.S1 = S1;
    g.tiles = air_cdiv(g.M, 16) * air_cdiv(A, 8);
    g.raw_offset = raw_offset; g.pl = p_loc; g.ps = p_scale; g.guard = guard_eps;
    const size_t n_pack = (size_t)B * (T * 5 + S0 + S1);
    int pb = (int)((n_pack + PW_THREADS - 1) / PW_THREADS);
    if (pb > 256) pb = 256;
    if (pb < 1) pb = 1;
    if (precision == AIR_PREC_BF16) hipLaunchKernelGGL((what_head_kernel<true>), dim3(g.tiles + pb), dim3(256), 0, air_stream(stream), g);
    else hipLaunchKernelGGL((what_head_kernel<false>), dim3(g.tiles + pb), dim3(256), 0, air_stream(stream), g);
    AIR_LAUNCH_CHECK();
    return AIR_OK;
}

template <bool BF>
__global__ __launch_bounds__(512) void lstm_fwd_wide_kernel(LstmFwdArgs g, PrologueArgs pro) {
    constexpr int KW = 8, LDT = 256 + 4;
    __shared__ float s_tile[KW][16 * LDT];
    if ((int)blockIdx.x >= g.tiles) {
        if (threadIdx.x < PW_THREADS) step_prologue_body(pro, (int)blockIdx.x - g.tiles, (int)gridDim.x - g.tiles);
        return;
    }
    const int lane = threadIdx.x & 63, wave = threadIdx.x >> 6, li = lane & 15, lg = lane >> 4;
    const int tiles_u = g.Hd >> 6;
    const int tm = blockIdx.x / tiles_u, tu = blockIdx.x - tm * tiles_u;
    const int m0 = tm * 16, u0 = tu * 64;
    const gcf gA = (gcf)g.h_prev, gW = (gcf)g.w_h;
    int rowA = m0 + li; if (rowA > g.M - 1) rowA = g.M - 1;
    const size_t offA = (size_t)rowA * g.ldh;
    const int colb = u0 + 4 * li;
    float e_gx[2][4], e_c[2];
#pragma unroll
    for (int i = 0; i < 2; ++i) {
        const int e = threadIdx.x + 512 * i, r = e >> 6, u = e & 63;
        int m = m0 + r; if (m > g.M - 1) m = g.M - 1;
        const gcf gx = (gcf)g.gx + (size_t)m * g.ldgx + u0 + u;
#pragma unroll
        for (int q = 0; q < 4; ++q) e_gx[i][q] = gx[(size_t)q * g.Hd];
        e_c[i] = ((gcf)g.c_prev)[(size_t)m * g.ldc + u0 + u];
    }
    f32x4 acc[16];
#pragma unroll
    for (int t = 0; t < 16; ++t) acc[t] = (f32x4){0.f, 0.f, 0.f, 0.f};
    constexpr int U = 2;
    const int nchunks = g.Hd >> 4;
#pragma nounroll
    for (int c = wave; c < nchunks; c += U * KW) {
        f32x4 fa[U], fw[U][4][4];
#pragma unroll
        for (int u = 0; u < U; ++u) {
            int cu = c + u * KW; if (cu > nchunks - 1) cu = nchunks - 1;
            const int k = (cu << 4) + 4 * lg;
            fa[u] = *(gcf4)(gA + offA + k);
#pragma unroll
            for (int j = 0; j < 4; ++j)
#pragma unroll
                for (int q = 0; q < 4; ++q) fw[u][j][q] = *(gcf4)(gW + (size_t)(k + j) * g.ldw + (size_t)q * g.Hd + colb);
        }
#pragma unroll
        for (int u = 0; u < U; ++u) {
            if (c + u * KW >= nchunks) break;
            if (BF) {
                const s16x4 ha = to_bf16x4(fa[u]);
#pragma unroll
                for (int q = 0; q < 4; ++q)
#pragma unroll
                    for (int cc = 0; cc < 4; ++cc) {
                        const s16x4 hb = to_bf16x4((f32x4){fw[u][0][q][cc], fw[u][1][q][cc], fw[u][2][q][cc], fw[u][3][q][cc]});
                        acc[q * 4 + cc] = __builtin_amdgcn_mfma_f32_16x16x16bf16_1k(ha, hb, acc[q * 4 + cc], 0, 0, 0);
                    }
            } else {
#pragma unroll
                for (int j = 0; j < 4; ++j)
#pragma unroll
                    for (int q = 0; q < 4; ++q)
#pragma unroll
                        for (int cc = 0; cc < 4; ++cc)
                            acc[q * 4 + cc] = __builtin_amdgcn_mfma_f32_16x16x4f32(fa[u][j], fw[u][j][q][cc], acc[q * 4 + cc], 0, 0, 0);
            }
        }
    }
#pragma unroll
    for (int q = 0; q < 4; ++q)
#pragma unroll
        for (int r = 0; r < 4; ++r)
            *(f32x4 *)&s_tile[wave][(4 * lg + r) * LDT + q * 64 + 4 * li] =
                (f32x4){acc[q * 4 + 0][r], acc[q * 4 + 1][r], acc[q * 4 + 2][r], acc[q * 4 + 3][r]};
    __syncthreads();
#pragma unroll
    for (int i = 0; i < 2; ++i) {
        const int e = threadIdx.x + 512 * i, r = e >> 6, u = e & 63;
        const int m = m0 + r;
        float pre[4];
#pragma unroll
        for (int q = 0; q < 4; ++q) {
            const int off = r * LDT + q * 64 + u;
            float v = 0.f;
#pragma unroll
            for (int w4 = 0; w4 < KW; w4 += 4)
                v += (s_tile[w4][off] + s_tile[w4 + 1][off]) + (s_tile[w4 + 2][off] + s_tile[w4 + 3][off]);
            pre[q] = v + e_gx[i][q];
        }
        if (m < g.M) {
            const float gi = sigmoid_acc(pre[0]);
            const float gj = tanhf(pre[1]);
            const float gf = sigmoid_acc(pre[2] + g.fb);
            const float go = sigmoid_acc(pre[3]);
            const float cn = gf * e_c[i] + gi * gj;
            const size_t eo = (size_t)m * g.Hd + u0 + u;
            ((gf_t)g.c)[eo] = cn;
            ((gf_t)g.h)[eo] = tanhf(cn) * go;
            const gf_t ar = (gf_t)g.gate_act + (size_t)m * 4 * g.Hd + u0 + u;
            ar[0] = gi; ar[g.Hd] = gj; ar[2 * (size_t)g.Hd] = gf; ar[3 * (size_t)g.Hd] = go;
        }
    }
}

struct LstmBwdArgs {
    const float *dgates_next, *w_h, *dh_a, *dh_b, *dc_in, *gate_act, *c_prev, *c, *dgx_in;
    float *dgates, *dc_prev, *dgx_out;
    int M, Hd, vecA, vecB;
};
template <int KW, bool BF>
__global__ __launch_bounds__(64 * KW) void lstm_bwd_fused_kernel(LstmBwdArgs g, RmspropSlice opt) {
    constexpr int LDT = 20;
    __shared__ float s_tile[KW][16 * LDT];
    const int lane = threadIdx.x & 63, wave = threadIdx.x >> 6, li = lane & 15, lg = lane >> 4;
    const int tiles_n = (g.Hd + 15) >> 4;
    {
        const int tiles = ((g.M + 15) >> 4) * tiles_n;
        if ((int)blockIdx.x >= tiles) {
            rmsprop_slice_body(opt, (int)blockIdx.x - tiles, (int)gridDim.x - tiles);
            return;
        }
    }
    const int tm = blockIdx.x / tiles_n, tn = blockIdx.x - tm * tiles_n;
    const int m0 = tm * 16, n0 = tn * 16;
    const int rowA = m0 + li, colB = n0 + li;
    const bool okA = rowA < g.M, okB = colB < g.Hd;
    const int K = 4 * g.Hd;
    const int er = threadIdx.x >> 4, ec = threadIdx.x & 15, em = m0 + er, eu = n0 + ec;
    const bool e_ok = threadIdx.x < 256 && em < g.M && eu < g.Hd;
    float gi = 0.f, gj = 0.f, gff = 0.f, go = 0.f, cp = 0.f, cc = 0.f, dha = 0.f, dhb = 0.f, dci = 0.f, sx[4] = {0.f, 0.f, 0.f, 0.f};
    if (e_ok) {
        const size_t e = (size_t)em * g.Hd + eu;
        const gcf ar = (gcf)g.gate_act + (size_t)em * K + eu;
        gi = ar[0]; gj = ar[g.Hd]; gff = ar[2 * (size_t)g.Hd]; go = ar[3 * (size_t)g.Hd];
        cp = ((gcf)g.c_prev)[e];
        cc = ((gcf)g.c)[e];
        if (g.dh_a) dha = ((gcf)g.dh_a)[e];
        if (g.dh_b) dhb = ((gcf)g.dh_b)[e];
        if (g.dc_in) dci = ((gcf)g.dc_in)[e];
        if (g.dgx_in) {
            const gcf sr = (gcf)g.dgx_in + (size_t)em * K + eu;
#pragma unroll
            for (int q = 0; q < 4; ++q) sx[q] = sr[(size_t)q * g.Hd];
        }
    }
    f32x4 acc[1][1];
    acc[0][0] = (f32x4){0.f, 0.f, 0.f, 0.f};
    tile16_kloop<KW, BF, true>(acc, (gcf)g.dgates_next, K, rowA, okA, g.vecA != 0, (gcf)g.w_h, K, colB, okB, g.vecB != 0, K,
                               g.M, g.Hd - 1);
#pragma unroll
    for (int r = 0; r < 4; ++r) s_tile[wave][(4 * lg + r) * LDT + li] = acc[0][0][r];
    __syncthreads();
    if (e_ok) {
        const int off = er * LDT + ec;
        float v = 0.f;
#pragma unroll
        for (int q = 0; q < KW; q += 4)
            v += (s_tile[q][off] + s_tile[q + 1][off]) + (s_tile[q + 2][off] + s_tile[q + 3][off]);
        const float dh = (v + dha) + dhb;
        const float tc = tanhf(cc);
        const float dct = dci + dh * go * (1.f - tc * tc);
        float d[4];
        d[0] = dct * gj * gi * (1.f - gi);
        d[1] = dct * gi * (1.f - gj * gj);
        d[2] = dct * cp * gff * (1.f - gff);
        d[3] = dh * tc * go * (1.f - go);
        const gf_t dr = (gf_t)g.dgates + (size_t)em * K + eu;
#pragma unroll
        for (int q = 0; q < 4; ++q) dr[(size_t)q * g.Hd] = d[q];
        ((gf_t)g.dc_prev)[(size_t)em * g.Hd + eu] = dct * gff;
        if (g.dgx_out) {
            const gf_t so = (gf_t)g.dgx_out + (size_t)em * K + eu;
#pragma unroll
            for (int q = 0; q < 4; ++q) so[(size_t)q * g.Hd] = sx[q] + d[q];
        }
    }
}

struct LstmEntryArgs {
    const float *gate_act1, *c_prev1, *c1, *dh_a1, *dh_b1;
    float *dgates1, *dc_prev1;
};
__device__ __forceinline__ void lstm_pw_bwd_elem(float gi, float gj, float gf, float go, float cp, float c, float dha, float dhb,
                                                 float dci, float (&d)[4], float &dc_prev) {
#pragma clang fp contract(off)
#ifdef AIR_LSTM_ENTRY_TANHF
    const float tc = tanhf(c);
#else
    const float tc = 1.f - __fdividef(2.f, __expf(2.f * c) + 1.f);
#endif
    const float dhe = dha + dhb;
    const float dct = dci + dhe * go * (1.f - tc * tc);
    d[0] = dct * gj * gi * (1.f - gi);
    d[1] = dct * gi * (1.f - gj * gj);
    d[2] = dct * cp * gf * (1.f - gf);
    d[3] = dhe * tc * go * (1.f - go);
    dc_prev = dct * gf;
}
__global__ __launch_bounds__(1024) void lstm_bwd_entry_kernel(LstmBwdArgs g, LstmEntryArgs en, RmspropSlice opt) {
    constexpr int KW = 16, LDT = 20;
    __shared__ float s_tile[KW][16 * LDT];
    const int lane = threadIdx.x & 63, wave = threadIdx.x >> 6, li = lane & 15, lg = lane >> 4;
    const int tiles_n = g.Hd >> 4;
    {
        const int tiles = ((g.M + 15) >> 4) * tiles_n;
        if ((int)blockIdx.x >= tiles) {
            rmsprop_slice_body(opt, (int)blockIdx.x - tiles, (int)gridDim.x - tiles);
            return;
        }
    }
    const int tm = blockIdx.x / tiles_n, tn = blockIdx.x - tm * tiles_n;
    const int m0 = tm * 16, n0 = tn * 16;
    const int rowA = m0 + li, colB = n0 + li;
    const bool okA = rowA < g.M;
    const int rowAc = okA ? rowA : g.M - 1;
    const int Hd = g.Hd, K = 4 * Hd;
    const int er = threadIdx.x >> 4, ec = threadIdx.x & 15, em = m0 + er, eu = n0 + ec;
    const bool e_ok = threadIdx.x < 256 && em < g.M;
    float gi = 0.f, gj = 0.f, gff = 0.f, go = 0.f, cp = 0.f, cc = 0.f, dha = 0.f, dhb = 0.f;
    float gi1 = 0.f, gj1 = 0.f, gf1 = 0.f, go1 = 0.f, cp1 = 0.f, cc1 = 0.f, dha1 = 0.f, dhb1 = 0.f;
    if (e_ok) {
        const size_t e = (size_t)em * Hd + eu;
        const gcf ar = (gcf)g.gate_act + (size_t)em * K + eu;
        gi = ar[0]; gj = ar[Hd]; gff = ar[2 * (size_t)Hd]; go = ar[3 * (size_t)Hd];
        cp = ((gcf)g.c_prev)[e];
        cc = ((gcf)g.c)[e];
        if (g.dh_a) dha = ((gcf)g.dh_a)[e];
        if (g.dh_b) dhb = ((gcf)g.dh_b)[e];
        const gcf a1 = (gcf)en.gate_act1 + (size_t)em * K + eu;
        gi1 = a1[0]; gj1 = a1[Hd]; gf1 = a1[2 * (size_t)Hd]; go1 = a1[3 * (size_t)Hd];
        cp1 = ((gcf)en.c_prev1)[e];
        cc1 = ((gcf)en.c1)[e];
        if (en.dh_a1) dha1 = ((gcf)en.dh_a1)[e];
        if (en.dh_b1) dhb1 = ((gcf)en.dh_b1)[e];
    }
    f32x4 acc = (f32x4){0.f, 0.f, 0.f, 0.f};
    const int nuc = Hd >> 4;
    const gcf gW = (gcf)g.w_h + (size_t)colB * K;
#pragma nounroll
    for (int uc = wave; uc < nuc; uc += KW) {
        const int u4 = (uc << 4) + 4 * lg;
        const size_t eo = (size_t)rowAc * Hd + u4, ao = (size_t)rowAc * K + u4;
        f32x4 a_g[4], fb[4];
#pragma unroll
        for (int q = 0; q < 4; ++q) a_g[q] = *(gcf4)((gcf)en.gate_act1 + ao + (size_t)q * Hd);
        const f32x4 v_cp = *(gcf4)((gcf)en.c_prev1 + eo), v_c = *(gcf4)((gcf)en.c1 + eo);
        f32x4 v_da = (f32x4){0.f, 0.f, 0.f, 0.f}, v_db = v_da;
        if (en.dh_a1) v_da = *(gcf4)((gcf)en.dh_a1 + eo);
        if (en.dh_b1) v_db = *(gcf4)((gcf)en.dh_b1 + eo);
#pragma unroll
        for (int q = 0; q < 4; ++q) fb[q] = *(gcf4)(gW + (size_t)q * Hd + u4);
        f32x4 fa[4], v_dcp;
#pragma unroll
        for (int x = 0; x < 4; ++x) {
            float d[4], dcp;
            lstm_pw_bwd_elem(a_g[0][x], a_g[1][x], a_g[2][x], a_g[3][x], v_cp[x], v_c[x], v_da[x], v_db[x], 0.f, d, dcp);
            fa[0][x] = d[0]; fa[1][x] = d[1]; fa[2][x] = d[2]; fa[3][x] = d[3];
            v_dcp[x] = dcp;
        }
        if (tn == 0 && okA) {
#pragma unroll
            for (int q = 0; q < 4; ++q) *(f32x4 *)(en.dgates1 + ao + (size_t)q * Hd) = fa[q];
            *(f32x4 *)(en.dc_prev1 + eo) = v_dcp;
        }
#pragma unroll
        for (int q = 0; q < 4; ++q)
#pragma unroll
            for (int j = 0; j < 4; ++j) acc = __builtin_amdgcn_mfma_f32_16x16x4f32(fa[q][j], fb[q][j], acc, 0, 0, 0);
    }
#pragma unroll
    for (int r = 0; r < 4; ++r) s_tile[wave][(4 * lg + r) * LDT + li] = acc[r];
    __syncthreads();
    if (e_ok) {
        const int off = er * LDT + ec;
        float v = 0.f;
#pragma unroll
        for (int q = 0; q < KW; q += 4)
            v += (s_tile[q][off] + s_tile[q + 1][off]) + (s_tile[q + 2][off] + s_tile[q + 3][off]);
        float d1[4], dci;
        lstm_pw_bwd_elem(gi1, gj1, gf1, go1, cp1, cc1, dha1, dhb1, 0.f, d1, dci);
        float d[4], dcp;
        lstm_pw_bwd_elem(gi, gj, gff, go, cp, cc, v + dha, dhb, dci, d, dcp);
        const gf_t dr = (gf_t)g.dgates + (size_t)em * K + eu;
#pragma unroll
        for (int q = 0; q < 4; ++q) dr[(size_t)q * Hd] = d[q];
        ((gf_t)g.dc_prev)[(size_t)em * Hd + eu] = dcp;
        if (g.dgx_out) {
            const gf_t so = (gf_t)g.dgx_out + (size_t)em * K + eu;
#pragma unroll
            for (int q = 0; q < 4; ++q) so[(size_t)q * Hd] = d1[q] + d[q];
        }
    }
}

template <bool BF>
__global__ __launch_bounds__(512) void lstm_bwd_wide_kernel(LstmBwdArgs g, RmspropSlice opt) {
    constexpr int KW = 8, NT = 4, LDT = 64 + 4;
    __shared__ float s_tile[KW][16 * LDT];
    const int tiles_n = g.Hd >> 6;
    {
        const int tiles = ((g.M + 15) >> 4) * tiles_n;
        if ((int)blockIdx.x >= tiles) {
            rmsprop_slice_body(opt, (int)blockIdx.x - tiles, (int)gridDim.x - tiles);
            return;
        }
    }
    const int lane = threadIdx.x & 63, wave = threadIdx.x >> 6, li = lane & 15, lg = lane >> 4;
    const int tm = blockIdx.x / tiles_n, tn = blockIdx.x - tm * tiles_n;
    const int m0 = tm * 16, n0 = tn * 64;
    const int K = 4 * g.Hd;
    const gcf gA = (gcf)g.dgates_next, gB = (gcf)g.w_h;
    int rowA = m0 + li; if (rowA > g.M - 1) rowA = g.M - 1;
    const size_t offA = (size_t)rowA * K;
    size_t offB[NT];
#pragma unroll
    for (int b = 0; b < NT; ++b) offB[b] = (size_t)(n0 + 16 * b + li) * K;
    float gi[2], gj[2], gff[2], go[2], cp[2], cc[2], dha[2], dhb[2], dci[2], sx[2][4];
#pragma unroll
    for (int i = 0; i < 2; ++i) {
        const int e_ = threadIdx.x + 512 * i, r = e_ >> 6, u = n0 + (e_ & 63);
        int m = m0 + r; if (m > g.M - 1) m = g.M - 1;
        const size_t e = (size_t)m * g.Hd + u;
        const gcf ar = (gcf)g.gate_act + (size_t)m * K + u;
        gi[i] = ar[0]; gj[i] = ar[g.Hd]; gff[i] = ar[2 * (size_t)g.Hd]; go[i] = ar[3 * (size_t)g.Hd];
        cp[i] = ((gcf)g.c_prev)[e];
        cc[i] = ((gcf)g.c)[e];
        dha[i] = g.dh_a ? ((gcf)g.dh_a)[e] : 0.f;
        dhb[i] = g.dh_b ? ((gcf)g.dh_b)[e] : 0.f;
        dci[i] = g.dc_in ? ((gcf)g.dc_in)[e] : 0.f;
#pragma unroll
        for (int q = 0; q < 4; ++q) sx[i][q] = g.dgx_in ? ((gcf)g.dgx_in)[(size_t)m * K + u + (size_t)q * g.Hd] : 0.f;
    }
    f32x4 acc[1][NT];
#pragma unroll
    for (int b = 0; b < NT; ++b) acc[0][b] = (f32x4){0.f, 0.f, 0.f, 0.f};
    constexpr int U = 4;
    const int nchunks = K >> 4;
#pragma nounroll
    for (int c = wave; c < nchunks; c += U * KW) {
        f32x4 fa[U][1], fb[U][NT];
#pragma unroll
        for (int u = 0; u < U; ++u) {
            int cu = c + u * KW; if (cu > nchunks - 1) cu = nchunks - 1;
            const int k = (cu << 4) + 4 * lg;
            fa[u][0] = *(gcf4)(gA + offA + k);
#pragma unroll
            for (int b = 0; b < NT; ++b) fb[u][b] = *(gcf4)(gB + offB[b] + k);
        }
#pragma unroll
        for (int u = 0; u < U; ++u) {
            if (c + u * KW >= nchunks) break;
            mfma_chunk<1, NT, BF>(acc, fa[u], fb[u]);
        }
    }
#pragma unroll
    for (int r = 0; r < 4; ++r)
#pragma unroll
        for (int b = 0; b < NT; ++b) s_tile[wave][(4 * lg + r) * LDT + 16 * b + li] = acc[0][b][r];
    __syncthreads();
#pragma unroll
    for (int i = 0; i < 2; ++i) {
        const int e_ = threadIdx.x + 512 * i, r = e_ >> 6, uc = e_ & 63, u = n0 + uc, m = m0 + r;
        const int off = r * LDT + uc;
        float v = 0.f;
#pragma unroll
        for (int q = 0; q < KW; q += 4) v += (s_tile[q][off] + s_tile[q + 1][off]) + (s_tile[q + 2][off] + s_tile[q + 3][off]);
        if (m >= g.M) continue;
        const float dh = (v + dha[i]) + dhb[i];
        const float tc = tanhf(cc[i]);
        const float dct = dci[i] + dh * go[i] * (1.f - tc * tc);
        float d[4];
        d[0] = dct * gj[i] * gi[i] * (1.f - gi[i]);
        d[1] = dct * gi[i] * (1.f - gj[i] * gj[i]);
        d[2] = dct * cp[i] * gff[i] * (1.f - gff[i]);
        d[3] = dh * tc * go[i] * (1.f - go[i]);
        const gf_t dr = (gf_t)g.dgates + (size_t)m * K + u;
#pragma unroll
        for (int q = 0; q < 4; ++q) dr[(size_t)q * g.Hd] = d[q];
        ((gf_t)g.dc_prev)[(size_t)m * g.Hd + u] = dct * gff[i];
        if (g.dgx_out) {
            const gf_t so = (gf_t)g.dgx_out + (size_t)m * K + u;
#pragma unroll
            for (int q = 0; q < 4; ++q) so[(size_t)q * g.Hd] = sx[i][q] + d[q];
        }
    }
}

struct Lstm16 { const void *w16, *a16; void *out16, *out16_b; };
__global__ __launch_bounds__(512) void lstm_fwd_wide16_kernel(LstmFwdArgs g, Lstm16 x) {
    constexpr int KW = 8, LDT = 256 + 4;
    __shared__ float s_tile[KW][16 * LDT];
    const int lane = threadIdx.x & 63, wave = threadIdx.x >> 6, li = lane & 15, lg = lane >> 4;
    const int tiles_u = g.Hd >> 6;
    const int tm = blockIdx.x / tiles_u, tu = blockIdx.x - tm * tiles_u;
    const int m0 = tm * 16, u0 = tu * 64;
    const gcf gA = (gcf)g.h_prev;
    const gch hA = (gch)x.a16, hW = (gch)x.w16;
    int rowA = m0 + li; if (rowA > g.M - 1) rowA = g.M - 1;
    const size_t offA = (size_t)rowA * g.ldh;
    const int colb = u0 + 4 * li;
    float e_gx[2][4], e_c[2];
#pragma unroll
    for (int i = 0; i < 2; ++i) {
        const int e = threadIdx.x + 512 * i, r = e >> 6, u = e & 63;
// ... 137 lines not shown
#pragma unroll
        for (int q = 0; q < KW; q += 4) v += (s_tile[q][off] + s_tile[q + 1][off]) + (s_tile[q + 2][off] + s_tile[q + 3][off]);
        if (m >= g.M) continue;
        const float dh = (v + dha[i]) + dhb[i];
        const float tc = tanhf(cc[i]);
        const float dct = dci[i] + dh * go[i] * (1.f - tc * tc);
        float d[4];
        d[0] = dct * gj[i] * gi[i] * (1.f - gi[i]);
        d[1] = dct * gi[i] * (1.f - gj[i] * gj[i]);
        d[2] = dct * cp[i] * gff[i] * (1.f - gff[i]);
        d[3] = dh * tc * go[i] * (1.f - go[i]);
        const gf_t dr = (gf_t)g.dgates + (size_t)m * K + u;
#pragma unroll
        for (int q = 0; q < 4; ++q) {
            dr[(size_t)q * g.Hd] = d[q];
            if (d16) d16[(size_t)m * K + u + (size_t)q * g.Hd] = bf16_bits(d[q]);
        }
        ((gf_t)g.dc_prev)[(size_t)m * g.Hd + u] = dct * gff[i];
        if (g.dgx_out) {
            const gf_t so = (gf_t)g.dgx_out + (size_t)m * K + u;
#pragma unroll
            for (int q = 0; q < 4; ++q) {
                const float sv = sx[i][q] + d[q];
                so[(size_t)q * g.Hd] = sv;
                if (s16) s16[(size_t)m * K + u + (size_t)q * g.Hd] = bf16_bits(sv);
            }
        }
    }
}

extern "C" int air_lstm_step_fwd_bf16(const float *h_prev, const void *h_prev_bf16, const float *c_prev, const void *w_h_bf16,
                                      int ldw, const float *gx, int ldgx, float *h, void *h_bf16, float *c, float *gate_act,
                                      int M, int Hd, float forget_bias, void *stream) {
    AIR_REQUIRE(h_prev && c_prev && w_h_bf16 && gx && h && c && gate_act, AIR_E_NULL);
    AIR_REQUIRE(M > 0 && Hd > 0 && Hd % 64 == 0 && ldw >= 4 * Hd && ldw % 4 == 0 && ldgx >= 4 * Hd, AIR_E_SHAPE);
    AIR_REQUIRE(air_aligned16(h_prev) && ((uintptr_t)w_h_bf16 % 8 == 0) && (!h_prev_bf16 || (uintptr_t)h_prev_bf16 % 16 == 0), AIR_E_ALIGN);
    LstmFwdArgs g;
    g.h_prev = h_prev; g.w_h = nullptr; g.gx = gx; g.c_prev = c_prev; g.h = h; g.c = c; g.gate_act = gate_act;
    g.M = M; g.Hd = Hd; g.ldw = ldw; g.ldgx = ldgx; g.vecA = 1; g.ldh = Hd; g.ldc = Hd; g.fb = forget_bias;
    g.tiles = air_cdiv(M, 16) * (Hd / 64);
    const Lstm16 x = {w_h_bf16, h_prev_bf16, h_bf16, nullptr};
    hipLaunchKernelGGL(lstm_fwd_wide16_kernel, dim3(g.tiles), dim3(512), 0, air_stream(stream), g, x);
    AIR_LAUNCH_CHECK();
    return AIR_OK;
}
extern "C" int air_lstm_step_bwd_bf16(const float *dgates_next, const void *dgates_next_bf16, const void *w_h_bf16,
                                      const float *dh_a, const float *dh_b, const float *dc_in, const float *gate_act,
                                      const float *c_prev, const float *c, const float *dgx_in, float *dgates,
                                      void *dgates_bf16, float *dc_prev, float *dgx_out, void *dgx_bf16, int M, int Hd,
                                      void *stream) {
    AIR_REQUIRE(dgates_next && w_h_bf16 && gate_act && c_prev && c && dgates && dc_prev, AIR_E_NULL);
    AIR_REQUIRE(M > 0 && Hd > 0 && Hd % 64 == 0, AIR_E_SHAPE);
    AIR_REQUIRE(air_aligned16(dgates_next) && ((uintptr_t)w_h_bf16 % 16 == 0) &&
                    (!dgates_next_bf16 || (uintptr_t)dgates_next_bf16 % 16 == 0), AIR_E_ALIGN);
    LstmBwdArgs g;
    g.dgates_next = dgates_next; g.w_h = nullptr; g.dh_a = dh_a; g.dh_b = dh_b; g.dc_in = dc_in; g.gate_act = gate_act;
    g.c_prev = c_prev; g.c = c; g.dgx_in = dgx_in; g.dgates = dgates; g.dc_prev = dc_prev; g.dgx_out = dgx_out;
    g.M = M; g.Hd = Hd; g.vecA = 1; g.vecB = 1;
    const Lstm16 x = {w_h_bf16, dgates_next_bf16, dgates_bf16, dgx_bf16};
    hipLaunchKernelGGL(lstm_bwd_wide16_kernel, dim3(air_cdiv(M, 16) * (Hd / 64)), dim3(512), 0, air_stream(stream), g, x);
    AIR_LAUNCH_CHECK();
    return AIR_OK;
}

template <bool BF>
static int lstm_fwd_launch(const LstmFwdArgs &g, const PrologueArgs &pro, int extra_blocks, hipStream_t st) {
    const bool wide = air_cdiv(g.M, 16) * air_cdiv(g.Hd, 16) > 512 && g.Hd % 64 == 0 && g.ldw % 4 == 0 && g.ldh % 4 == 0 &&
                      air_aligned16(g.w_h) && air_aligned16(g.h_prev);
    if (wide) {
        LstmFwdArgs gw = g;
        gw.tiles = air_cdiv(g.M, 16) * (g.Hd / 64);
        hipLaunchKernelGGL((lstm_fwd_wide_kernel<BF>), dim3(gw.tiles + extra_blocks), dim3(512), 0, st, gw, pro);
    } else {
        hipLaunchKernelGGL((lstm_fwd_fused_kernel<BF>), dim3(g.tiles + extra_blocks), dim3(256), 0, st, g, pro);
    }
    AIR_LAUNCH_CHECK();
    return AIR_OK;
}
static int lstm_fwd_fill(LstmFwdArgs &g, const float *h_prev, int ldh, const float *c_prev, int ldc, const float *w_h,
                         int ldw, const float *gx, int ldgx, float *h, float *c, float *gate_act, int M, int Hd,
                         float forget_bias, int precision) {
    AIR_REQUIRE(h_prev && c_prev && w_h && gx && h && c && gate_act, AIR_E_NULL);
    AIR_REQUIRE(M > 0 && Hd > 0 && ldw >= 4 * Hd && ldgx >= 4 * Hd, AIR_E_SHAPE);
    AIR_REQUIRE((ldh == 0 || ldh >= Hd) && (ldc == 0 || ldc >= Hd), AIR_E_SHAPE);
    AIR_REQUIRE(precision == AIR_PREC_F32 || precision == AIR_PREC_BF16, AIR_E_UNSUPPORTED);
    g.h_prev = h_prev; g.w_h = w_h; g.gx = gx; g.c_prev = c_prev; g.h = h; g.c = c; g.gate_act = gate_act;
    g.M = M; g.Hd = Hd; g.ldw = ldw; g.ldgx = ldgx; g.fb = forget_bias; g.ldh = ldh; g.ldc = ldc;
    g.vecA = ((ldh % 4) == 0 && air_aligned16(h_prev)) ? 1 : 0;
    g.tiles = air_cdiv(M, 16) * air_cdiv(Hd, 4);
    return AIR_OK;
}
extern "C" int air_lstm_step_fwd(const float *h_prev, const float *c_prev, const float *w_h, int ldw, const float *gx,
                                 int ldgx, float *h, float *c, float *gate_act, int M, int Hd, float forget_bias,
                                 int precision, void *stream) {
    LstmFwdArgs g;
    int st = lstm_fwd_fill(g, h_prev, Hd, c_prev, Hd, w_h, ldw, gx, ldgx, h, c, gate_act, M, Hd, forget_bias, precision);
    if (st) return st;
    PrologueArgs pro = {};
    return precision == AIR_PREC_BF16 ? lstm_fwd_launch<true>(g, pro, 0, air_stream(stream))
                                      : lstm_fwd_launch<false>(g, pro, 0, air_stream(stream));
}
extern "C" int air_lstm_step_fwd_prologue(const float *h0, const float *c0, const float *w_h, int ldw, const float *gx,
                                          int ldgx, float *h, float *c, float *gate_act, int M, int Hd, float forget_bias,
                                          int precision, float *normal, size_t n_normal, float *uniform, size_t n_uniform,
                                          const uint64_t *rng_state_dev, const int64_t *global_step_dev, int anneal_type,
                                          double init, double final_value, double anneal_steps, double hold_for,
                                          double steps_div, double *prior_out_f64, int T, float *h_tiled, float *c_tiled,
                                          void *stream) {
    AIR_REQUIRE(rng_state_dev && global_step_dev && prior_out_f64 && h_tiled && c_tiled, AIR_E_NULL);
    AIR_REQUIRE((n_normal == 0 || normal) && (n_uniform == 0 || uniform), AIR_E_NULL);
    AIR_REQUIRE(T > 0 && anneal_type >= 0 && anneal_type <= 2, AIR_E_SHAPE);
    LstmFwdArgs g;
    int st = lstm_fwd_fill(g, h0, 0, c0, 0, w_h, ldw, gx, ldgx, h, c, gate_act, M, Hd, forget_bias, precision);
    if (st) return st;
    const PrologueArgs pro = make_prologue_args(normal, n_normal, uniform, n_uniform, rng_state_dev, global_step_dev,
                                                anneal_type, init, final_value, anneal_steps, hold_for, steps_div,
                                                prior_out_f64, T, h0, c0, h_tiled, c_tiled, M, Hd);
    const int extra = prologue_blocks(pro);
    return precision == AIR_PREC_BF16 ? lstm_fwd_launch<true>(g, pro, extra, air_stream(stream))
                                      : lstm_fwd_launch<false>(g, pro, extra, air_stream(stream));
}

extern "C" int air_lstm_first_step_fwd(const float *x, int ldx, int E, const float *w_x, const float *b_gates, const float *h0,
                                       const float *c0, const float *w_h, int ldw, float *gx_out, int ldgx, float *h, float *c,
                                       float *gate_act, int M, int Hd, float forget_bias, int precision, float *normal,
                                       size_t n_normal, float *uniform, size_t n_uniform, const uint64_t *rng_state_dev,
                                       const int64_t *global_step_dev, int anneal_type, double init, double final_value,
                                       double anneal_steps, double hold_for, double steps_div, double *prior_out_f64, int T,
                                       float *h_tiled, float *c_tiled, void *stream) {
    AIR_REQUIRE(x && w_x && b_gates && gx_out, AIR_E_NULL);
    AIR_REQUIRE(rng_state_dev && global_step_dev && prior_out_f64 && h_tiled && c_tiled, AIR_E_NULL);
    AIR_REQUIRE((n_normal == 0 || normal) && (n_uniform == 0 || uniform), AIR_E_NULL);
    AIR_REQUIRE(T > 0 && anneal_type >= 0 && anneal_type <= 2 && E > 0 && ldx >= E, AIR_E_SHAPE);
    AIR_REQUIRE(air_cdiv(M, 16) * air_cdiv(Hd, 16) <= 512, AIR_E_UNSUPPORTED);
    AIR_REQUIRE(air_gemm_lone_on_tile16_kw4(M, 4 * Hd, E), AIR_E_UNSUPPORTED);
    LstmFwdArgs g;
    int st = lstm_fwd_fill(g, h0, 0, c0, 0, w_h, ldw, gx_out, ldgx, h, c, gate_act, M, Hd, forget_bias, precision);
    if (st) return st;
    LstmFirstArgs f;
    f.x = x; f.w_x = w_x; f.b = b_gates; f.gx_out = gx_out; f.E = E; f.ldx = ldx;
    f.vecX = ((ldx % 4) == 0 && air_aligned16(x)) ? 1 : 0;
    const PrologueArgs pro = make_prologue_args(normal, n_normal, uniform, n_uniform, rng_state_dev, global_step_dev,
                                                anneal_type, init, final_value, anneal_steps, hold_for, steps_div,
                                                prior_out_f64, T, h0, c0, h_tiled, c_tiled, M, Hd);
    const int extra = prologue_blocks(pro);
    if (precision == AIR_PREC_BF16)
        hipLaunchKernelGGL((lstm_fwd_first_kernel<true>), dim3(g.tiles + extra), dim3(256), 0, air_stream(stream), g, f, pro);
    else
        hipLaunchKernelGGL((lstm_fwd_first_kernel<false>), dim3(g.tiles + extra), dim3(256), 0, air_stream(stream), g, f, pro);
    AIR_LAUNCH_CHECK();
    return AIR_OK;
}

template <bool BF>
static int lstm_bwd_launch(const LstmBwdArgs &g, const RmspropSlice &opt, size_t opt_nq, hipStream_t st) {
    const int tiles = air_cdiv(g.M, 16) * air_cdiv(g.Hd, 16);
    const bool wide = tiles > 512 && g.Hd % 64 == 0 && g.vecA && g.vecB;
    const int nth = tiles <= 512 ? 1024 : (wide ? 512 : 256);
    size_t extra = air_rider_blocks(opt_nq, nth, 512);
    if (wide) hipLaunchKernelGGL((lstm_bwd_wide_kernel<BF>), dim3(air_cdiv(g.M, 16) * (g.Hd / 64) + (int)extra), dim3(512), 0, st, g, opt);
    else if (tiles <= 512) hipLaunchKernelGGL((lstm_bwd_fused_kernel<16, BF>), dim3(tiles + (int)extra), dim3(1024), 0, st, g, opt);
    else hipLaunchKernelGGL((lstm_bwd_fused_kernel<4, BF>), dim3(tiles + (int)extra), dim3(256), 0, st, g, opt);
    AIR_LAUNCH_CHECK();
    return AIR_OK;
}
extern "C" int air_lstm_step_bwd(const float *dgates_next, const float *w_h, const float *dh_a, const float *dh_b,
                                 const float *dc_in, const float *gate_act, const float *c_prev, const float *c,
                                 const float *dgx_in, float *dgates, float *dc_prev, float *dgx_out, int M, int Hd,
                                 int precision, void *stream) {
    return air_lstm_step_bwd_opt(dgates_next, w_h, dh_a, dh_b, dc_in, gate_act, c_prev, c, dgx_in, dgates, dc_prev, dgx_out, M,
                                 Hd, precision, nullptr, stream);
}
extern "C" int air_lstm_step_bwd_opt(const float *dgates_next, const float *w_h, const float *dh_a, const float *dh_b,
                                     const float *dc_in, const float *gate_act, const float *c_prev, const float *c,
                                     const float *dgx_in, float *dgates, float *dc_prev, float *dgx_out, int M, int Hd,
                                     int precision, const AirRmspropSlice *opt, void *stream) {
    RmspropSlice os; size_t onq;
    { int st_ = rmsprop_slice_from_abi(opt, os, &onq); if (st_) return st_; }
    AIR_REQUIRE(dgates_next && w_h && gate_act && c_prev && c && dgates && dc_prev, AIR_E_NULL);
    AIR_REQUIRE(M > 0 && Hd > 0, AIR_E_SHAPE);
    AIR_REQUIRE(precision == AIR_PREC_F32 || precision == AIR_PREC_BF16, AIR_E_UNSUPPORTED);
    LstmBwdArgs g;
    g.dgates_next = dgates_next; g.w_h = w_h; g.dh_a = dh_a; g.dh_b = dh_b; g.dc_in = dc_in; g.gate_act = gate_act;
    g.c_prev = c_prev; g.c = c; g.dgx_in = dgx_in; g.dgates = dgates; g.dc_prev = dc_prev; g.dgx_out = dgx_out;
    g.M = M; g.Hd = Hd;
    g.vecA = air_aligned16(dgates_next) ? 1 : 0;
    g.vecB = air_aligned16(w_h) ? 1 : 0;
    return precision == AIR_PREC_BF16 ? lstm_bwd_launch<true>(g, os, onq, air_stream(stream))
                                      : lstm_bwd_launch<false>(g, os, onq, air_stream(stream));
}

extern "C" int air_lstm_step_bwd_entry_fits(int M, int Hd) {
    return (M > 0 && Hd > 0 && Hd % 16 == 0 && air_cdiv(M, 16) * (Hd / 16) <= 512) ? 1 : 0;
}
extern "C" int air_lstm_step_bwd_entry(const float *gate_act1, const float *c_prev1, const float *c1, const float *dh_a1,
                                       const float *dh_b1, float *dgates1, float *dc_prev1, const float *w_h, const float *dh_a,
                                       const float *dh_b, const float *gate_act, const float *c_prev, const float *c, float *dgates,
                                       float *dc_prev, float *dgx_out, int M, int Hd, const AirRmspropSlice *opt, void *stream) {
    RmspropSlice os; size_t onq;
    { int st_ = rmsprop_slice_from_abi(opt, os, &onq); if (st_) return st_; }
    AIR_REQUIRE(gate_act1 && c_prev1 && c1 && dgates1 && dc_prev1 && w_h && gate_act && c_prev && c && dgates && dc_prev, AIR_E_NULL);
    AIR_REQUIRE(dh_a1 || dh_b1, AIR_E_NULL);
    AIR_REQUIRE(air_lstm_step_bwd_entry_fits(M, Hd) == 1, AIR_E_UNSUPPORTED);
    AIR_REQUIRE(air_aligned16(gate_act1) && air_aligned16(c_prev1) && air_aligned16(c1) && air_aligned16(dgates1) &&
                air_aligned16(dc_prev1) && air_aligned16(w_h) && (!dh_a1 || air_aligned16(dh_a1)) && (!dh_b1 || air_aligned16(dh_b1)),
                AIR_E_ALIGN);
    LstmBwdArgs g;
    g.dgates_next = dgates1; g.w_h = w_h; g.dh_a = dh_a; g.dh_b = dh_b; g.dc_in = nullptr; g.gate_act = gate_act;
    g.c_prev = c_prev; g.c = c; g.dgx_in = nullptr; g.dgates = dgates; g.dc_prev = dc_prev; g.dgx_out = dgx_out;
    g.M = M; g.Hd = Hd; g.vecA = 1; g.vecB = 1;
    LstmEntryArgs en;
    en.gate_act1 = gate_act1; en.c_prev1 = c_prev1; en.c1 = c1; en.dh_a1 = dh_a1; en.dh_b1 = dh_b1; en.dgates1 = dgates1;
    en.dc_prev1 = dc_prev1;
    const int tiles = air_cdiv(M, 16) * (Hd / 16);
    size_t extra = air_rider_blocks(onq, 1024, 512);
    hipLaunchKernelGGL(lstm_bwd_entry_kernel, dim3(tiles + (int)extra), dim3(1024), 0, air_stream(stream), g, en, os);
    AIR_LAUNCH_CHECK();
    return AIR_OK;
}
```

### attend_infer_repeat_amd/gemm_groups.py

```python
from . import _lib

GROUPED, SPLITK = "grouped", "splitk"


def tiles16(d):
    return ((d.M + 15) // 16) * ((d.N + 15) // 16)


def is_weight_gradient(d):
    return bool(d.ta and not d.tb)


def wide_ok(d, group_tiles16):
    strict = group_tiles16 > 2048 or (d.A % 16 == 0 and d.lda % 4 == 0 and d.K % 4 == 0)
    return bool(strict and not (d.ta and d.tb) and not d.A2 and d.B % 16 == 0 and d.ldb % 4 == 0
                and (not (d.ta or d.tb) or d.K % 4 == 0) and d.M >= 4 and d.N >= 4 and d.K >= 4
                and (not d.ta or d.M % 4 == 0) and (d.tb or d.N % 4 == 0))


def plan_launch(descs, throughput, use16, allow_splitk=False):
    total = sum(tiles16(d) for d in descs)
    if throughput and len(descs) > 1:
        ok = [wide_ok(d, total) for d in descs]
        if any(ok) and not all(ok):
# ... 137 lines not shown
        return False
    for d in descs:
        off = (int(d.A) - obs) // 4
        if d.ta or d.A2 or d.C16 or d.precision != 0 or d.M != B or d.lda != item_floats:
            return False
        if (int(d.A) - obs) % 4 or off < 0 or off + d.K > item_floats or off % 4:
            return False
    return on_long_k_body(descs, wide_min_tiles)


def tensors_read(descs, p0, p1, spans):
    out = []
    for d in descs:
        for x in (d.A, d.B, d.aux, d.bias, d.A2):
            if p0 <= int(x or 0) < p1:
                off = (int(x) - p0) // 4
                out += [sp for sp in spans if sp[0] <= off < sp[1]]
    return out


def foldable(descs, g0, r_lo, barred):
    mask, cov = 0, []
    for i, d in enumerate(descs):
        if not is_weight_gradient(d):
            continue
        off = (int(d.C) - g0) // 4
        if not (0 <= off < r_lo) or d.ldc != d.N or d.beta != 0.0 or d.epilogue != 0:
            continue
        mine = [(off, off + d.M * d.N)]
        if d.colsum:
            coff = (int(d.colsum) - g0) // 4
            mine.append((coff, coff + d.N))
        if any(a0 < b1 and b0 < a1 for a0, a1 in mine for b0, b1 in barred):
            continue
        mask |= 1 << i
        cov += mine
    return mask, cov


E_NULL, E_SHAPE, E_ALIGN, E_UNSUPPORTED = -1, -2, -3, -5
FORM_FIELDS = tuple(n for n, _ in _lib.AirGemmForm._fields_)


def _form(**kw):
    f = dict.fromkeys(FORM_FIELDS, 0)
    f.update({k: int(v) for k, v in kw.items()})
    return f


def _cdiv(a, b):
    return (a + b - 1) // b


def _a(p):
    return int(p or 0)


def single_form(M, N, K, colsum=False, ws_bytes=0):
    if M <= 0 or N <= 0 or K <= 0:
        return E_SHAPE, None
    chunks = _cdiv(K, 16)
    if _cdiv(M, 32) * _cdiv(N, 32) >= 2048:
        return 0, _form(family=0, MT=2, NT=2, KW=1, tile=32, S=1, chunks_per_split=chunks, workgroups=_cdiv(M, 32) * _cdiv(N, 128), threads=256)
    tiles = _cdiv(M, 16) * _cdiv(N, 16)
    S = 1
    if not colsum and ws_bytes > 0 and chunks >= 64:
        s = min(1024 // tiles, chunks // 16, ws_bytes // (M * N * 4), 16)
        if s >= 2:
            S = s
    cps = _cdiv(chunks, S)
    return 0, _form(family=0, MT=1, NT=1, KW=4, tile=16, S=_cdiv(chunks, cps), chunks_per_split=cps, workgroups=tiles, threads=256)


def _desc_status(d):
    if not (_a(d.A) and _a(d.B) and _a(d.C)):
        return E_NULL
    if not (d.M > 0 and d.N > 0 and d.K > 0):
        return E_SHAPE
    if not (d.lda >= (d.M if d.ta else d.K) and d.ldb >= (d.K if d.tb else d.N) and d.ldc >= d.N):
        return E_SHAPE
    if not 0 <= d.epilogue <= 5:
        return E_UNSUPPORTED
    if d.epilogue in (1, 2) and not _a(d.bias):
        return E_NULL
    if d.epilogue >= 3 and not (_a(d.aux) and d.ldaux >= d.N):
        return E_NULL
    if _a(d.colsum) and not d.ta:
        return E_UNSUPPORTED
    if _a(d.A2):
        if d.ta or not _a(d.a_bias) or d.K % 16 or d.lda % 4:
            return E_UNSUPPORTED
        if _a(d.A) % 16 or _a(d.A2) % 16 or _a(d.a_bias) % 16 or _a(d.a_out) % 16:
            return E_ALIGN
    return 0


def _mirror_usable(m16, ld):
    return bool(_a(m16) and ld % 2 == 0 and _a(m16) % 4 == 0)


def _big_tn_form(descs, bf16_storage, big_xcd):
    if len(descs) > 24:
        return E_SHAPE, None
    bf = descs[0].precision == 1
    f = _form(grouped=1, MT=4, KW=8, bf=bf, ta=1, threads=512)
    min_k, n_wide = 1 << 30, 0
    for i, d in enumerate(descs):
        if d.precision not in (0, 1) or (d.precision == 1) != bf or _a(d.A2):
            return E_UNSUPPORTED, None
        st = _desc_status(d)
        if st:
            return st, None
        if (d.ta and not d.tb and _a(d.B) % 16 == 0 and d.ldb % 4 == 0 and d.K % 4 == 0 and d.M >= 4 and d.N >= 4 and d.M % 4 == 0
                and d.N % 4 == 0):
            min_k, n_wide = min(min_k, d.K), n_wide + 1
            f["workgroups"] += _cdiv(d.M, 64) * _cdiv(d.N, 64)
        else:
            f["small_mask"] |= 1 << i
            f["workgroups"] += _cdiv(d.M, 16) * _cdiv(d.N, 16)
        if bf and bf16_storage and _mirror_usable(d.A16, d.lda):
            f["a16_mask"] |= 1 << i
        if bf and bf16_storage and _mirror_usable(d.B16, d.ldb):
            f["b16_mask"] |= 1 << i
    if not n_wide:
        return E_UNSUPPORTED, None
    f["xcd_map"] = ((2 if bf else 1) if (big_xcd and min_k >= 1024) else 0)
    f["family"] = 7 if bf else 6
    return 0, f


def wide_group_eligible(descs, bf, wide_min_tiles=1000, wide_tn_bf16=48, wide_tn_f32=48, wide_nt_k=512):
    t16 = sum(tiles16(d) for d in descs)
    ok = t16 > wide_min_tiles
    ta, tb = bool(descs[0].ta), bool(descs[0].tb)
    tiles64, min_k = 0, 1 << 30
    for d in descs:
        if not ok:
            break
        ok = bool(d.ta) == ta and bool(d.tb) == tb and not (ta and tb) and not _a(d.A2)
        ok = ok and _a(d.B) % 16 == 0 and d.ldb % 4 == 0 and (not ta or d.K % 4 == 0) and (not tb or d.K % 4 == 0)
        ok = ok and d.M >= 4 and d.N >= 4 and d.K >= 4 and (not ta or d.M % 4 == 0) and (tb or d.N % 4 == 0)
        if t16 <= 2048:
            ok = ok and _a(d.A) % 16 == 0 and d.lda % 4 == 0 and d.K % 4 == 0
        tiles64 += _cdiv(d.M, 64) * _cdiv(d.N, 64)
        min_k = min(min_k, d.K)
    if ok and ta:
        ok = tiles64 >= (wide_tn_bf16 if bf else wide_tn_f32) and min_k >= 256
    nt_short = (not ta) and tb and min_k < wide_nt_k
    if ok and nt_short:
        ok = bf and t16 > 2048
    return bool(ok), min_k, bool(nt_short)


def grouped_form(descs, wide_min_tiles=1000, shortk=True, shortk_min_m=4096, shortk_wgs=384, wide_tn_bf16=48, wide_tn_f32=48, wide_nt_k=512,
                 bf16_storage=True, big_xcd=True):
    count = len(descs)
    if count > 8:
        return _big_tn_form(descs, bf16_storage, big_xcd)
    if count <= 0:
        return E_SHAPE, None

    def validate():
        for d in descs:
            st = _desc_status(d)
            if st:
                return st
        return 0

    skm = 0
    if shortk and not any(_a(d.A2) or _a(d.C16) or d.precision != 0 for d in descs):
        skm = sum(1 << i for i, d in enumerate(descs) if shortk_eligible(d, shortk_min_m))
    if skm:
        st = validate()
        if st:
            return st, None
        tile = latency_tile(sum(tiles16(d) for i, d in enumerate(descs) if not (skm >> i) & 1))
        wgs = sum(shortk_workgroups(d.M, shortk_wgs) if (skm >> i) & 1 else _cdiv(d.M, tile) * _cdiv(d.N, tile) for i, d in enumerate(descs))
        return 0, _form(family=3, grouped=1, sk_mask=skm, tile=tile, MT=tile // 16, NT=tile // 16, KW=4, threads=256, workgroups=wgs)
    t16 = sum(tiles16(d) for d in descs)
    tile = latency_tile(t16)
    st = validate()
    if st:
        return st, None
    lk = group_long_k(descs)
    bf = descs[0].precision == 1
    if any(d.precision not in (0, 1) or (d.precision == 1) != bf for d in descs):
        return E_UNSUPPORTED, None
    ok, min_k, nt_short = wide_group_eligible(descs, bf, wide_min_tiles, wide_tn_bf16, wide_tn_f32, wide_nt_k)
    ta, tb = bool(descs[0].ta), bool(descs[0].tb)
    if ok and bf and ta:
        return _big_tn_form(descs, bf16_storage, big_xcd)
    if ok:
        MT = 4 if ta else (2 if nt_short else 1)
        f = _form(family=5 if bf else 4, grouped=count > 1, bf=bf, ta=ta, tb=tb, nt_short=nt_short, MT=MT, KW=8, threads=512,
                  workgroups=sum(_cdiv(d.M, 16 * MT) * _cdiv(d.N, 64) for d in descs), xcd_map=ta and min_k >= 1024)
        if bf:
            full = (1 << count) - 1
            f["a16_mask"] = full if bf16_storage and all(_mirror_usable(d.A16, d.lda) for d in descs) else 0
            f["b16_mask"] = full if bf16_storage and all(_mirror_usable(d.B16, d.ldb) for d in descs) else 0
        return 0, f
    if any(_a(d.A2) for d in descs) and count != 1:
        return E_UNSUPPORTED, None
    mt = 1 if (lk or tile == 16) else 2
    f = _form(grouped=count > 1, bf=bf, tile=tile, long_k=lk, MT=mt, NT=mt, KW=16 if lk else 4, threads=1024 if lk else 256,
              workgroups=sum(_cdiv(d.M, tile) * _cdiv(d.N, tile) for d in descs))
    if any(_a(d.C16) for d in descs):
        if not bf or _a(descs[0].A2):
            return E_UNSUPPORTED, None
        f["family"] = 1
    elif count == 1 and _a(descs[0].A2):
        if tile != 16:
            return E_UNSUPPORTED, None
        f.update(family=2, MT=1, NT=1, KW=4, threads=256)
    return 0, f
```

Measured before the change: 315,400 images/sec.

## Use half-height 8x16 output tiles for small long-K GEMMs and LSTM backward

Adds a half-tile mode to the 16-wave long-K GEMM body and to the LSTM backward fused and entry kernels. Each workgroup owns 8x16 (or 8x8) outputs, with masked loads for the unused rows. When the 16x16 tile count would fill at most half the CUs, the workgroup count doubles so more CUs take part in the small, latency-bound batch-64 GEMMs. In exchange, half of each MFMA tile computes wasted lanes, B-operand traffic is duplicated across workgroups, and environment-variable overrides are added.

```diff
diff --git a/attend_infer_repeat_amd/csrc/air_common.h b/attend_infer_repeat_amd/csrc/air_common.h
--- a/attend_infer_repeat_amd/csrc/air_common.h
+++ b/attend_infer_repeat_amd/csrc/air_common.h
@@ -2,6 +2,7 @@
 #include <hip/hip_runtime.h>
 #include <stdint.h>
 #include <stdlib.h>
+#include <string.h>
 #include <mutex>
 #include "../../include/air_hip.h"
 
@@ -19,6 +20,42 @@
 static inline bool air_gemm_lone_on_tile16_kw4(int M, int N, int K) {
     const long t = (long)((M + 15) / 16) * ((N + 15) / 16);
     return t <= air_gemm_wide_min_tiles() && air_gemm_latency_tile(t) == 16 && !air_gemm_long_k(M, N, K);
+}
+
+enum { AIR_TILE_AUTO = 0, AIR_TILE_16x16, AIR_TILE_8x16, AIR_TILE_8x8, AIR_TILE_UNKNOWN };
+static inline int air_tile_shape(const char *e, size_t n) {
+    if (n == 0 || (n == 4 && !strncmp(e, "auto", 4))) return AIR_TILE_AUTO;
+    if (n == 5 && !strncmp(e, "16x16", 5)) return AIR_TILE_16x16;
+    if (n == 4 && !strncmp(e, "8x16", 4)) return AIR_TILE_8x16;
+    if (n == 3 && !strncmp(e, "8x8", 3)) return AIR_TILE_8x8;
+    return AIR_TILE_UNKNOWN;
+}
+static inline int air_tile_env(const char *name, const char *key) {
+    const char *e = getenv(name);
+    if (!e) return AIR_TILE_AUTO;
+    if (!strchr(e, '=')) return air_tile_shape(e, strlen(e));
+    int shape = AIR_TILE_AUTO;
+    const size_t nk = strlen(key);
+    while (*e) {
+        const char *end = strchr(e, ',');
+        const size_t n = end ? (size_t)(end - e) : strlen(e);
+        const char *eq = (const char *)memchr(e, '=', n);
+        if (!eq) return AIR_TILE_UNKNOWN;
+        const int s = air_tile_shape(eq + 1, n - (size_t)(eq + 1 - e));
+        if (s == AIR_TILE_UNKNOWN) return s;
+        if ((size_t)(eq - e) == nk && !strncmp(e, key, nk)) shape = s;
+        e += n + (end ? 1 : 0);
+    }
+    return shape;
+}
+static inline int air_cu_count() {
+    static const int cus = [] {
+        int dev = 0, n = 0;
+        if (hipGetDevice(&dev) != hipSuccess || hipDeviceGetAttribute(&n, hipDeviceAttributeMultiprocessorCount, dev) != hipSuccess || n < 1)
+            n = 256;
+        return n;
+    }();
+    return cus;
 }
 
 static inline hipStream_t air_stream(void *s) { return reinterpret_cast<hipStream_t>(s); }
diff --git a/attend_infer_repeat_amd/csrc/gemm_kernels.hip b/attend_infer_repeat_amd/csrc/gemm_kernels.hip
--- a/attend_infer_repeat_amd/csrc/gemm_kernels.hip
+++ b/attend_infer_repeat_amd/csrc/gemm_kernels.hip
@@ -100,10 +100,12 @@
     return v;
 }
 
-template <int MT, int NT, int KW, bool BF, bool APRO = false, bool OPT = false, bool GBW = false, bool GATH = false>
+template <int MT, int NT, int KW, bool BF, bool APRO = false, bool OPT = false, bool GBW = false, bool GATH = false, bool HALF = false>
 __device__ __forceinline__ void gemm_body(const GemmArgs &g, const int block_tile, const int split, const AproArgs pro = AproArgs(),
                                           void *c16 = nullptr, const OptFold *opt = nullptr, const bool fold = false,
-                                          const GaussEpi *gb = nullptr, const GatherArgs *gt = nullptr, const bool gcopy = false) {
+                                          const GaussEpi *gb = nullptr, const GatherArgs *gt = nullptr, const bool gcopy = false,
+                                          const int own_r = 16, const int own_c = 16) {
+    static_assert(!HALF || (MT == 1 && NT == 1 && KW == 16 && !APRO && !OPT && !GBW && !GATH), "half tiles: the plain 16-wave body only");
     const gh_t hC = (gh_t)c16;
     constexpr int TM = 16 * MT, TN = 16 * NT;
     constexpr int NWN = (KW == 1) ? 4 : 1;
@@ -117,10 +119,12 @@
     const gf gC = (gf)g.C, gWs = (gf)g.ws, gCol = (gf)g.colsum;
     const int lane = threadIdx.x & 63, wave = threadIdx.x >> 6;
     const int li = lane & 15, lg = lane >> 4;
-    const int tiles_n = (g.N + TN * NWN - 1) / (TN * NWN);
+    const int OWN_M = HALF ? own_r : TM, OWN_N = HALF ? own_c : TN;
+    const int tiles_n = (g.N + OWN_N * NWN - 1) / (OWN_N * NWN);
     const int tm = block_tile / tiles_n, tn = block_tile - tm * tiles_n;
-    const int m0 = tm * TM;
-    const int n0 = (tn * NWN + (KW == 1 ? wave : 0)) * TN;
+    const int m0 = tm * OWN_M;
+    const int n0 = (tn * NWN + (KW == 1 ? wave : 0)) * OWN_N;
+    const int own_sh = own_c == 8 ? 3 : 4;
 
     const int total_chunks = (g.K + 15) >> 4;
     const int c_begin = split * g.chunks_per_split;
@@ -140,9 +144,9 @@
     int rowA[MT], colB[NT];
     bool okA[MT], okB[NT];
 #pragma unroll
-    for (int a = 0; a < MT; ++a) { rowA[a] = m0 + 16 * a + li; okA[a] = rowA[a] < g.M; }
-#pragma unroll
-    for (int b = 0; b < NT; ++b) { colB[b] = n0 + 16 * b + li; okB[b] = colB[b] < g.N; }
+    for (int a = 0; a < MT; ++a) { rowA[a] = m0 + 16 * a + li; okA[a] = rowA[a] < g.M && (!HALF || li < own_r); }
+#pragma unroll
+    for (int b = 0; b < NT; ++b) { colB[b] = n0 + 16 * b + li; okB[b] = colB[b] < g.N && (!HALF || li < own_c); }
 
     constexpr int EPT = (KW > 1) ? (TM * TN + NTH - 1) / NTH : 1;
     float e_bias[EPT], e_aux[EPT], e_c[EPT];
@@ -150,9 +154,9 @@
 #pragma unroll
         for (int i = 0; i < EPT; ++i) {
             const int e = threadIdx.x + NTH * i;
-            const int r = e / TN, cidx = e - r * TN;
+            const int r = HALF ? (e >> own_sh) : e / TN, cidx = e - r * OWN_N;
             const int m = m0 + r, n = n0 + cidx;
-            const bool ok = (e < TM * TN) && m < g.M && n < g.N;
+            const bool ok = (e < OWN_M * OWN_N) && m < g.M && n < g.N;
             e_bias[i] = (ok && g.bias != nullptr) ? gBias[n] : 0.f;
             e_aux[i] = (ok && g.epi >= AIR_EPI_MUL_DELU) ? gAux[(size_t)m * g.ldaux + n] : 0.f;
             e_c[i] = (ok && g.beta != 0.f) ? gC[(size_t)m * g.ldc + n] : 0.f;
@@ -163,9 +167,9 @@
 #pragma unroll
         for (int i = 0; i < EPT; ++i) {
             const int e = threadIdx.x + NTH * i;
-            const int r = e / TN, cidx = e - r * TN;
+            const int r = HALF ? (e >> own_sh) : e / TN, cidx = e - r * OWN_N;
             const int m = m0 + r, n = n0 + cidx;
-            const bool ok = (e < TM * TN) && m < g.M && n < g.N;
+            const bool ok = (e < OWN_M * OWN_N) && m < g.M && n < g.N;
             const size_t o = ok ? (size_t)m * gb->D + n : 0;
             b_loc[i] = ok ? ((gcf)gb->loc)[o] : 0.f;
             b_scale[i] = ok ? ((gcf)gb->scale)[o] : 1.f;
@@ -181,9 +185,9 @@
 #pragma unroll
         for (int i = 0; i < EPT; ++i) {
             const int e = threadIdx.x + NTH * i;
-            const int r = e / TN, cidx = e - r * TN;
+            const int r = HALF ? (e >> own_sh) : e / TN, cidx = e - r * OWN_N;
             const int m = m0 + r, n = n0 + cidx;
-            const bool ok = (e < TM * TN) && m < g.M && n < g.N;
+            const bool ok = (e < OWN_M * OWN_N) && m < g.M && n < g.N;
             const size_t idx = ok ? (size_t)((gC + (size_t)m * g.ldc + n) - (gf)opt->g0) : 0;
             o_p[i] = ok ? ((gf)opt->p)[idx] : 0.f;
             o_ms[i] = ok ? ((gf)opt->ms)[idx] : 0.f;
@@ -223,6 +227,7 @@
                 const int k = (cu << 4) + 4 * lg;
 #pragma unroll
                 for (int a = 0; a < MT; ++a) {
+                    if (HALF && !okA[a]) { fa[u][a] = (f32x4){0.f, 0.f, 0.f, 0.f}; continue; }
                     fa[u][a] = g.ta ? ld_kstrided_full(gA, g.lda, rowAc[a], k)
                                     : ld_kcontig_full(gAs, ldAs, rowAs[a], k, g.vecA != 0);
                     if (APRO) {
@@ -231,9 +236,11 @@
                     }
                 }
 #pragma unroll
-                for (int b = 0; b < NT; ++b)
+                for (int b = 0; b < NT; ++b) {
+                    if (HALF && !okB[b]) { fb[u][b] = (f32x4){0.f, 0.f, 0.f, 0.f}; continue; }
                     fb[u][b] = g.tb ? ld_kcontig_full(gB, g.ldb, colBc[b], k, g.vecB != 0)
                                     : ld_kstrided_full(gB, g.ldb, colBc[b], k);
+                }
             } else {
 #pragma unroll
                 for (int a = 0; a < MT; ++a) fa[u][a] = (f32x4){0.f, 0.f, 0.f, 0.f};
@@ -318,8 +325,8 @@
 #pragma unroll
         for (int i = 0; i < EPT; ++i) {
             const int e = threadIdx.x + NTH * i;
-            if (e >= TM * TN) continue;
-            const int r = e / TN, cidx = e - r * TN;
+            if (e >= OWN_M * OWN_N) continue;
+            const int r = HALF ? (e >> own_sh) : e / TN, cidx = e - r * OWN_N;
             const int m = m0 + r, n = n0 + cidx;
             if (m >= g.M || n >= g.N) continue;
             const int off = r * LDT + cidx;
@@ -874,6 +881,15 @@
 #undef AIR_GG_CASE
 }
 
+__global__ __launch_bounds__(1024) void gemm_grouped_longk_half_kernel(GroupArgs ga, unsigned own8) {
+#define AIR_GH_CASE(I_)                                                                                                              \
+    gemm_body<1, 1, 16, false, false, false, false, false, true>(ga.g[I_], (int)blockIdx.x - ga.tile_start[I_], blockIdx.y, AproArgs(),  \
+                                                                 nullptr, nullptr, false, nullptr, nullptr, false,                  \
+                                                                 ((own8 >> (2 * I_)) & 1u) ? 8 : 16, ((own8 >> (2 * I_ + 1)) & 1u) ? 8 : 16)
+    AIR_GROUP_DISPATCH(ga, (int)blockIdx.x, AIR_GH_CASE);
+#undef AIR_GH_CASE
+}
+
 __global__ __launch_bounds__(1024) void gemm_grouped_gather_kernel(GroupArgs ga, GatherArgs gt) {
 #define AIR_GG_CASE(I_)                                                                                                             \
     gemm_body<1, 1, 16, false, false, false, false, true>(ga.g[I_], (int)blockIdx.x - ga.tile_start[I_], blockIdx.y, AproArgs(), nullptr, \
@@ -1383,7 +1399,7 @@
         if (int st = fill_gemm_args(scratch, descs[i])) return st;
     return AIR_OK;
 }
-static int form_workgroups_of(const AirGemmForm &f, int i, const AirGemmDesc &d) {
+static int form_workgroups_of(const AirGemmForm &f, int i, const AirGemmDesc &d, unsigned own8 = 0u) {
     switch (f.family) {
         case AIR_GEMM_FAM_BIG: case AIR_GEMM_FAM_BIG16:
             return ((f.small_mask >> i) & 1u) ? air_cdiv(d.M, 16) * air_cdiv(d.N, 16) : air_cdiv(d.M, 64) * air_cdiv(d.N, 64);
@@ -1393,12 +1409,30 @@
             if ((f.sk_mask >> i) & 1u) return shortk_workgroups(d.M);
             [[fallthrough]];
         default:
-            return air_cdiv(d.M, f.tile) * air_cdiv(d.N, f.tile);
-    }
-}
-static void form_sum_workgroups(AirGemmForm &f, const AirGemmDesc *descs, int count) {
+            return air_cdiv(d.M, ((own8 >> (2 * i)) & 1u) ? 8 : f.tile) * air_cdiv(d.N, ((own8 >> (2 * i + 1)) & 1u) ? 8 : f.tile);
+    }
+}
+static void form_sum_workgroups(AirGemmForm &f, const AirGemmDesc *descs, int count, unsigned own8 = 0u) {
     f.workgroups = 0;
-    for (int i = 0; i < count; ++i) f.workgroups += form_workgroups_of(f, i, descs[i]);
+    for (int i = 0; i < count; ++i) f.workgroups += form_workgroups_of(f, i, descs[i], own8);
+}
+static constexpr bool GEMM_LONGK_TILE_AUTO = true;
+static int longk_half_shapes(const AirGemmDesc *descs, int count, const AirGemmForm &f, long tiles16, unsigned *own8) {
+    *own8 = 0u;
+    if (f.family != AIR_GEMM_FAM_TILE || f.KW != 16) return AIR_OK;
+    int shape = air_tile_env("AIR_GEMM_LONGK_TILE", "group");
+    AIR_REQUIRE(shape != AIR_TILE_UNKNOWN, AIR_E_UNSUPPORTED);
+    bool domain = !f.bf;
+    for (int i = 0; i < count; ++i)
+        domain = domain && !descs[i].ta && descs[i].tb && !descs[i].colsum &&
+                 (descs[i].epilogue == AIR_EPI_NONE || descs[i].epilogue == AIR_EPI_MUL_DELU);
+    AIR_REQUIRE(domain || shape == AIR_TILE_AUTO || shape == AIR_TILE_16x16, AIR_E_UNSUPPORTED);
+    if (shape == AIR_TILE_AUTO) {
+        shape = (GEMM_LONGK_TILE_AUTO && domain && count > 1 && 2 * tiles16 <= air_cu_count()) ? AIR_TILE_8x16 : AIR_TILE_16x16;
+    }
+    const unsigned per = shape == AIR_TILE_8x8 ? 3u : (shape == AIR_TILE_8x16 ? 1u : 0u);
+    for (int i = 0; i < count; ++i) *own8 |= per << (2 * i);
+    return AIR_OK;
 }
 static int big_tn_form(const AirGemmDesc *descs, int count, AirGemmForm &f) {
     AIR_REQUIRE(count <= AIR_GEMM_BIG_GROUP_MAX, AIR_E_SHAPE);
@@ -1501,8 +1535,9 @@
     return AIR_OK;
 }
 
-static int gemm_grouped_form(const AirGemmDesc *descs, int count, AirGemmForm &f) {
+static int gemm_grouped_form(const AirGemmDesc *descs, int count, AirGemmForm &f, unsigned *own8_out = nullptr) {
     memset(&f, 0, sizeof f);
+    if (own8_out) *own8_out = 0u;
     if (count > AIR_GEMM_GROUP_MAX) return big_tn_form(descs, count, f);
     AIR_REQUIRE(count > 0 && count <= AIR_GEMM_GROUP_MAX, AIR_E_SHAPE);
     f.grouped = count > 1 ? 1 : 0;
@@ -1560,7 +1595,11 @@
         AIR_REQUIRE(T_ == 16, AIR_E_UNSUPPORTED);
         f.family = AIR_GEMM_FAM_APRO; f.MT = f.NT = 1; f.KW = 4; f.threads = 256;
     } else f.family = AIR_GEMM_FAM_TILE;
-    form_sum_workgroups(f, descs, count);
+    unsigned own8;
+    if (int err = longk_half_shapes(descs, count, f, tiles16, &own8)) return err;
+    if (own8) { f.grouped = 1; f.small_mask = (1u << count) - 1u; }
+    if (own8_out) *own8_out = own8;
+    form_sum_workgroups(f, descs, count, own8);
     return AIR_OK;
 }
 extern "C" int air_gemm_grouped_form(const AirGemmDesc *descs, int count, AirGemmForm *out) {
@@ -1571,16 +1610,22 @@
 extern "C" int air_gemm_grouped(const AirGemmDesc *descs, int count, void *stream) {
     AIR_REQUIRE(descs, AIR_E_NULL);
     AirGemmForm f;
-    if (int err = gemm_grouped_form(descs, count, f)) return err;
+    unsigned own8 = 0u;
+    if (int err = gemm_grouped_form(descs, count, f, &own8)) return err;
     if (f.family == AIR_GEMM_FAM_BIG || f.family == AIR_GEMM_FAM_BIG16) return launch_big_tn_group(descs, count, f, stream);
     if (f.family == AIR_GEMM_FAM_SHORTK) return launch_grouped_sk(descs, count, f, stream);
     GroupArgs ga;
     int tiles = 0;
     const bool wide = f.family == AIR_GEMM_FAM_WIDE || f.family == AIR_GEMM_FAM_WIDE16;
-    int err = fill_group(ga, descs, count, accept_any, [&](int i, const AirGemmDesc &d) { return form_workgroups_of(f, i, d); }, &tiles);
+    int err = fill_group(ga, descs, count, accept_any, [&](int i, const AirGemmDesc &d) { return form_workgroups_of(f, i, d, own8); }, &tiles);
     if (err) return err;
     hipStream_t st = air_stream(stream);
     const bool bf = f.bf != 0;
+    if (own8) {
+        hipLaunchKernelGGL(gemm_grouped_longk_half_kernel, dim3(tiles), dim3(1024), 0, st, ga, own8);
+        AIR_LAUNCH_CHECK();
+        return AIR_OK;
+    }
     if (wide) {
         const int wt = tiles;
         ga.xcd_map = f.xcd_map;
diff --git a/attend_infer_repeat_amd/csrc/lstm_kernels.hip b/attend_infer_repeat_amd/csrc/lstm_kernels.hip
--- a/attend_infer_repeat_amd/csrc/lstm_kernels.hip
+++ b/attend_infer_repeat_amd/csrc/lstm_kernels.hip
@@ -5,7 +5,7 @@
 #include "nvil_device.h"
 #include "gemm_device.h"
 
-template <int KW, bool BF, bool B_KCONTIG>
+template <int KW, bool BF, bool B_KCONTIG, bool MASK = false>
 __device__ __forceinline__ void tile16_kloop(f32x4 (&acc)[1][1], gcf gA, int lda, int rowA, bool okA, bool vecA, gcf gB,
                                              int ldb, int colB, bool okB, bool vecB, int K, int limA, int limB) {
     const int lane = threadIdx.x & 63, wave = threadIdx.x >> 6, lg = lane >> 4;
@@ -20,8 +20,10 @@
             const int cu = c + u * KW;
             if (cu < full_end) {
                 const int k = (cu << 4) + 4 * lg;
-                fa[u][0] = ld_kcontig_full(gA, lda, rowAc, k, vecA);
-                fb[u][0] = B_KCONTIG ? ld_kcontig_full(gB, ldb, colBc, k, vecB) : ld_kstrided_full(gB, ldb, colBc, k);
+                fa[u][0] = (f32x4){0.f, 0.f, 0.f, 0.f};
+                fb[u][0] = (f32x4){0.f, 0.f, 0.f, 0.f};
+                if (!MASK || okA) fa[u][0] = ld_kcontig_full(gA, lda, rowAc, k, vecA);
+                if (!MASK || okB) fb[u][0] = B_KCONTIG ? ld_kcontig_full(gB, ldb, colBc, k, vecB) : ld_kstrided_full(gB, ldb, colBc, k);
             } else {
                 fa[u][0] = (f32x4){0.f, 0.f, 0.f, 0.f};
                 fb[u][0] = (f32x4){0.f, 0.f, 0.f, 0.f};
@@ -407,26 +409,26 @@
     float *dgates, *dc_prev, *dgx_out;
     int M, Hd, vecA, vecB;
 };
-template <int KW, bool BF>
+template <int KW, bool BF, int R = 16, int C = 16>
 __global__ __launch_bounds__(64 * KW) void lstm_bwd_fused_kernel(LstmBwdArgs g, RmspropSlice opt) {
     constexpr int LDT = 20;
     __shared__ float s_tile[KW][16 * LDT];
     const int lane = threadIdx.x & 63, wave = threadIdx.x >> 6, li = lane & 15, lg = lane >> 4;
-    const int tiles_n = (g.Hd + 15) >> 4;
+    const int tiles_n = (g.Hd + C - 1) / C;
     {
-        const int tiles = ((g.M + 15) >> 4) * tiles_n;
+        const int tiles = ((g.M + R - 1) / R) * tiles_n;
         if ((int)blockIdx.x >= tiles) {
             rmsprop_slice_body(opt, (int)blockIdx.x - tiles, (int)gridDim.x - tiles);
             return;
         }
     }
     const int tm = blockIdx.x / tiles_n, tn = blockIdx.x - tm * tiles_n;
-    const int m0 = tm * 16, n0 = tn * 16;
+    const int m0 = tm * R, n0 = tn * C;
     const int rowA = m0 + li, colB = n0 + li;
-    const bool okA = rowA < g.M, okB = colB < g.Hd;
+    const bool okA = li < R && rowA < g.M, okB = li < C && colB < g.Hd;
     const int K = 4 * g.Hd;
-    const int er = threadIdx.x >> 4, ec = threadIdx.x & 15, em = m0 + er, eu = n0 + ec;
-    const bool e_ok = threadIdx.x < 256 && em < g.M && eu < g.Hd;
+    const int er = threadIdx.x / C, ec = threadIdx.x & (C - 1), em = m0 + er, eu = n0 + ec;
+    const bool e_ok = threadIdx.x < R * C && em < g.M && eu < g.Hd;
     float gi = 0.f, gj = 0.f, gff = 0.f, go = 0.f, cp = 0.f, cc = 0.f, dha = 0.f, dhb = 0.f, dci = 0.f, sx[4] = {0.f, 0.f, 0.f, 0.f};
     if (e_ok) {
         const size_t e = (size_t)em * g.Hd + eu;
@@ -445,8 +447,8 @@
     }
     f32x4 acc[1][1];
     acc[0][0] = (f32x4){0.f, 0.f, 0.f, 0.f};
-    tile16_kloop<KW, BF, true>(acc, (gcf)g.dgates_next, K, rowA, okA, g.vecA != 0, (gcf)g.w_h, K, colB, okB, g.vecB != 0, K,
-                               g.M, g.Hd - 1);
+    tile16_kloop<KW, BF, true, (R < 16 || C < 16)>(acc, (gcf)g.dgates_next, K, rowA, okA, g.vecA != 0, (gcf)g.w_h, K, colB, okB, g.vecB != 0, K,
+                                                   g.M, g.Hd - 1);
 #pragma unroll
     for (int r = 0; r < 4; ++r) s_tile[wave][(4 * lg + r) * LDT + li] = acc[0][0][r];
     __syncthreads();
@@ -496,26 +498,27 @@
     d[3] = dhe * tc * go * (1.f - go);
     dc_prev = dct * gf;
 }
+template <int R, int C>
 __global__ __launch_bounds__(1024) void lstm_bwd_entry_kernel(LstmBwdArgs g, LstmEntryArgs en, RmspropSlice opt) {
     constexpr int KW = 16, LDT = 20;
     __shared__ float s_tile[KW][16 * LDT];
     const int lane = threadIdx.x & 63, wave = threadIdx.x >> 6, li = lane & 15, lg = lane >> 4;
-    const int tiles_n = g.Hd >> 4;
+    const int tiles_n = g.Hd / C;
     {
-        const int tiles = ((g.M + 15) >> 4) * tiles_n;
+        const int tiles = ((g.M + R - 1) / R) * tiles_n;
         if ((int)blockIdx.x >= tiles) {
             rmsprop_slice_body(opt, (int)blockIdx.x - tiles, (int)gridDim.x - tiles);
             return;
         }
     }
     const int tm = blockIdx.x / tiles_n, tn = blockIdx.x - tm * tiles_n;
-    const int m0 = tm * 16, n0 = tn * 16;
-    const int rowA = m0 + li, colB = n0 + li;
-    const bool okA = rowA < g.M;
-    const int rowAc = okA ? rowA : g.M - 1;
+    const int m0 = tm * R, n0 = tn * C;
+    const int rowA = m0 + li, colB = n0 + (li & (C - 1));
+    const bool okA = li < R && rowA < g.M, okB = li < C;
+    const int rowAc = rowA < g.M ? rowA : g.M - 1;
     const int Hd = g.Hd, K = 4 * Hd;
-    const int er = threadIdx.x >> 4, ec = threadIdx.x & 15, em = m0 + er, eu = n0 + ec;
-    const bool e_ok = threadIdx.x < 256 && em < g.M;
+    const int er = threadIdx.x / C, ec = threadIdx.x & (C - 1), em = m0 + er, eu = n0 + ec;
+    const bool e_ok = threadIdx.x < R * C && em < g.M;
     float gi = 0.f, gj = 0.f, gff = 0.f, go = 0.f, cp = 0.f, cc = 0.f, dha = 0.f, dhb = 0.f;
     float gi1 = 0.f, gj1 = 0.f, gf1 = 0.f, go1 = 0.f, cp1 = 0.f, cc1 = 0.f, dha1 = 0.f, dhb1 = 0.f;
     if (e_ok) {
@@ -541,14 +544,21 @@
         const int u4 = (uc << 4) + 4 * lg;
         const size_t eo = (size_t)rowAc * Hd + u4, ao = (size_t)rowAc * K + u4;
         f32x4 a_g[4], fb[4];
-#pragma unroll
-        for (int q = 0; q < 4; ++q) a_g[q] = *(gcf4)((gcf)en.gate_act1 + ao + (size_t)q * Hd);
-        const f32x4 v_cp = *(gcf4)((gcf)en.c_prev1 + eo), v_c = *(gcf4)((gcf)en.c1 + eo);
-        f32x4 v_da = (f32x4){0.f, 0.f, 0.f, 0.f}, v_db = v_da;
-        if (en.dh_a1) v_da = *(gcf4)((gcf)en.dh_a1 + eo);
-        if (en.dh_b1) v_db = *(gcf4)((gcf)en.dh_b1 + eo);
-#pragma unroll
-        for (int q = 0; q < 4; ++q) fb[q] = *(gcf4)(gW + (size_t)q * Hd + u4);
+        const f32x4 zero4 = (f32x4){0.f, 0.f, 0.f, 0.f};
+        f32x4 v_cp = zero4, v_c = zero4, v_da = zero4, v_db = zero4;
+#pragma unroll
+        for (int q = 0; q < 4; ++q) { a_g[q] = zero4; fb[q] = zero4; }
+        if (R == 16 || okA) {
+#pragma unroll
+            for (int q = 0; q < 4; ++q) a_g[q] = *(gcf4)((gcf)en.gate_act1 + ao + (size_t)q * Hd);
+            v_cp = *(gcf4)((gcf)en.c_prev1 + eo); v_c = *(gcf4)((gcf)en.c1 + eo);
+            if (en.dh_a1) v_da = *(gcf4)((gcf)en.dh_a1 + eo);
+            if (en.dh_b1) v_db = *(gcf4)((gcf)en.dh_b1 + eo);
+        }
+        if (C == 16 || okB) {
+#pragma unroll
+            for (int q = 0; q < 4; ++q) fb[q] = *(gcf4)(gW + (size_t)q * Hd + u4);
+        }
         f32x4 fa[4], v_dcp;
 #pragma unroll
         for (int x = 0; x < 4; ++x) {
@@ -992,13 +1002,28 @@
     return AIR_OK;
 }
 
+enum { LSTM_LINK_TILE = AIR_TILE_8x16, LSTM_ENTRY_TILE = AIR_TILE_8x16 };
+static int lstm_bwd_tile_auto(int M, int Hd, int adopted) {
+    const long tiles16 = (long)air_cdiv(M, 16) * air_cdiv(Hd, 16);
+    return (2 * tiles16 > air_cu_count() || 4 * Hd < 512) ? (int)AIR_TILE_16x16 : adopted;
+}
+
 template <bool BF>
 static int lstm_bwd_launch(const LstmBwdArgs &g, const RmspropSlice &opt, size_t opt_nq, hipStream_t st) {
     const int tiles = air_cdiv(g.M, 16) * air_cdiv(g.Hd, 16);
     const bool wide = tiles > 512 && g.Hd % 64 == 0 && g.vecA && g.vecB;
     const int nth = tiles <= 512 ? 1024 : (wide ? 512 : 256);
     size_t extra = air_rider_blocks(opt_nq, nth, 512);
+    int shape = air_tile_env("AIR_LSTM_BWD_TILE", "link");
+    AIR_REQUIRE(shape != AIR_TILE_UNKNOWN, AIR_E_UNSUPPORTED);
+    AIR_REQUIRE(shape == AIR_TILE_AUTO || shape == AIR_TILE_16x16 || (tiles <= 512 && !BF), AIR_E_UNSUPPORTED);
+    if (shape == AIR_TILE_AUTO)
+        shape = (tiles <= 512 && !BF) ? lstm_bwd_tile_auto(g.M, g.Hd, LSTM_LINK_TILE) : AIR_TILE_16x16;
     if (wide) hipLaunchKernelGGL((lstm_bwd_wide_kernel<BF>), dim3(air_cdiv(g.M, 16) * (g.Hd / 64) + (int)extra), dim3(512), 0, st, g, opt);
+    else if (shape == AIR_TILE_8x16)
+        hipLaunchKernelGGL((lstm_bwd_fused_kernel<16, false, 8, 16>), dim3(air_cdiv(g.M, 8) * air_cdiv(g.Hd, 16) + (int)extra), dim3(1024), 0, st, g, opt);
+    else if (shape == AIR_TILE_8x8)
+        hipLaunchKernelGGL((lstm_bwd_fused_kernel<16, false, 8, 8>), dim3(air_cdiv(g.M, 8) * air_cdiv(g.Hd, 8) + (int)extra), dim3(1024), 0, st, g, opt);
     else if (tiles <= 512) hipLaunchKernelGGL((lstm_bwd_fused_kernel<16, BF>), dim3(tiles + (int)extra), dim3(1024), 0, st, g, opt);
     else hipLaunchKernelGGL((lstm_bwd_fused_kernel<4, BF>), dim3(tiles + (int)extra), dim3(256), 0, st, g, opt);
     AIR_LAUNCH_CHECK();
@@ -1052,9 +1077,16 @@
     LstmEntryArgs en;
     en.gate_act1 = gate_act1; en.c_prev1 = c_prev1; en.c1 = c1; en.dh_a1 = dh_a1; en.dh_b1 = dh_b1; en.dgates1 = dgates1;
     en.dc_prev1 = dc_prev1;
-    const int tiles = air_cdiv(M, 16) * (Hd / 16);
     size_t extra = air_rider_blocks(onq, 1024, 512);
-    hipLaunchKernelGGL(lstm_bwd_entry_kernel, dim3(tiles + (int)extra), dim3(1024), 0, air_stream(stream), g, en, os);
+    int shape = air_tile_env("AIR_LSTM_BWD_TILE", "entry");
+    AIR_REQUIRE(shape != AIR_TILE_UNKNOWN, AIR_E_UNSUPPORTED);
+    if (shape == AIR_TILE_AUTO) shape = lstm_bwd_tile_auto(M, Hd, LSTM_ENTRY_TILE);
+    if (shape == AIR_TILE_8x16)
+        hipLaunchKernelGGL((lstm_bwd_entry_kernel<8, 16>), dim3(air_cdiv(M, 8) * (Hd / 16) + (int)extra), dim3(1024), 0, air_stream(stream), g, en, os);
+    else if (shape == AIR_TILE_8x8)
+        hipLaunchKernelGGL((lstm_bwd_entry_kernel<8, 8>), dim3(air_cdiv(M, 8) * (Hd / 8) + (int)extra), dim3(1024), 0, air_stream(stream), g, en, os);
+    else
+        hipLaunchKernelGGL((lstm_bwd_entry_kernel<16, 16>), dim3(air_cdiv(M, 16) * (Hd / 16) + (int)extra), dim3(1024), 0, air_stream(stream), g, en, os);
     AIR_LAUNCH_CHECK();
     return AIR_OK;
 }
diff --git a/attend_infer_repeat_amd/gemm_groups.py b/attend_infer_repeat_amd/gemm_groups.py
--- a/attend_infer_repeat_amd/gemm_groups.py
+++ b/attend_infer_repeat_amd/gemm_groups.py
@@ -313,8 +313,14 @@
     return bool(ok), min_k, bool(nt_short)
 
 
+def longk_half_tile(descs, bf, cus=256, adopted=True):
+    t16 = sum(tiles16(d) for d in descs)
+    domain = not bf and all((not d.ta) and d.tb and not _a(d.colsum) and d.epilogue in (0, 3) for d in descs)
+    return (8, 16) if (adopted and domain and len(descs) > 1 and 2 * t16 <= cus) else (16, 16)
+
+
 def grouped_form(descs, wide_min_tiles=1000, shortk=True, shortk_min_m=4096, shortk_wgs=384, wide_tn_bf16=48, wide_tn_f32=48, wide_nt_k=512,
-                 bf16_storage=True, big_xcd=True):
+                 bf16_storage=True, big_xcd=True, cus=256):
     count = len(descs)
     if count > 8:
         return _big_tn_form(descs, bf16_storage, big_xcd)
@@ -373,4 +379,8 @@
         if tile != 16:
             return E_UNSUPPORTED, None
         f.update(family=2, MT=1, NT=1, KW=4, threads=256)
+    elif lk:
+        tr, tc = longk_half_tile(descs, bf, cus)
+        if (tr, tc) != (16, 16):
+            f.update(grouped=1, small_mask=(1 << count) - 1, workgroups=sum(_cdiv(d.M, tr) * _cdiv(d.N, tc) for d in descs))
     return 0, f
```

After: 320,300 images/sec, median of 6. 1.02x the previous value.
